# elasticdeeplearning/trainingjob-operator

Hardware: AMD Instinct MI355X
Metric: tokens_per_sec_llama3_8b (higher is better)
Workload: dtype bf16; 1 GPU; model=llama3-8b, global_batch=4, seq_len=4096, parallelism=dp1, micro_batch=2, grad_accum=2, checkpoint_activations=False

## Files before the change

### trainingjob_operator_amd/models/llama.py

```python
from __future__ import annotations

import math
import os
from typing import Optional

import torch
import torch.nn as nn
import torch.nn.functional as F


def _sdpa(q, k, v, enable_gqa=False, is_causal=True):
    backend = os.environ.get("AITJ_SDPA_BACKEND", "auto")
    if q.is_cuda and backend in ("auto", "native") and is_causal:
        from ..ops.attention import _supported, flash_attention
        qc = q.contiguous() if q.stride(-1) != 1 else q
        if _supported(qc, k):
            return flash_attention(qc, k, v)
        if backend == "native":
            groups = q.shape[1] // k.shape[1]
            if groups > 1:
                k = k.repeat_interleave(groups, dim=1)
                v = v.repeat_interleave(groups, dim=1)
            return flash_attention(qc, k, v)
    if backend in ("auto", "native") or not q.is_cuda:
        return F.scaled_dot_product_attention(q, k, v, is_causal=is_causal,
                                              enable_gqa=enable_gqa)
    from torch.nn.attention import SDPBackend, sdpa_kernel
    mapping = {"flash": SDPBackend.FLASH_ATTENTION,
               "efficient": SDPBackend.EFFICIENT_ATTENTION,
               "math": SDPBackend.MATH}
    with sdpa_kernel([mapping[backend]]):
        return F.scaled_dot_product_attention(q, k, v, is_causal=is_causal,
                                              enable_gqa=enable_gqa)

from ..ops import (apply_rope, fused_cross_entropy, fused_rmsnorm,
                   make_inv_freq, swiglu_packed)
from ..ops.fp8 import fp8_enabled, fp8_linear


def _proj(x, linear):
    if fp8_enabled() and x.is_cuda:
        return fp8_linear(x, linear)
    return linear(x)
from .config import LlamaConfig


class Attention(nn.Module):
    def __init__(self, cfg: LlamaConfig):
        super().__init__()
        self.cfg = cfg
        H = cfg.hidden_size
        self.q_size = cfg.num_heads * cfg.head_dim
        self.kv_size = cfg.num_kv_heads * cfg.head_dim
        self.qkv_proj = nn.Linear(H, self.q_size + 2 * self.kv_size,
                                  bias=False)
        self.o_proj = nn.Linear(self.q_size, H, bias=False)

    def forward(self, x: torch.Tensor, inv_freq: torch.Tensor) -> torch.Tensor:
        B, S, H = x.shape
        cfg = self.cfg
        qkv = _proj(x, self.qkv_proj)
        q, k, v = qkv.split([self.q_size, self.kv_size, self.kv_size],
                            dim=-1)
        q = q.reshape(B, S, cfg.num_heads, cfg.head_dim).contiguous()
        k = k.reshape(B, S, cfg.num_kv_heads, cfg.head_dim).contiguous()
        v = v.reshape(B, S, cfg.num_kv_heads, cfg.head_dim)
        q = apply_rope(q, inv_freq, S)
        k = apply_rope(k, inv_freq, S)
        q = q.transpose(1, 2)
        k = k.transpose(1, 2)
        v = v.transpose(1, 2)
        if cfg.num_heads != cfg.num_kv_heads and \
                os.environ.get("AITJ_DISABLE_GQA"):
            groups = cfg.num_heads // cfg.num_kv_heads
            k = k.repeat_interleave(groups, dim=1)
            v = v.repeat_interleave(groups, dim=1)
            o = _sdpa(q, k, v)
        else:
            o = _sdpa(q, k, v,
                      enable_gqa=cfg.num_heads != cfg.num_kv_heads)
        o = o.transpose(1, 2).reshape(B, S, cfg.num_heads * cfg.head_dim)
        return _proj(o, self.o_proj)


class MLP(nn.Module):
    def __init__(self, cfg: LlamaConfig):
        super().__init__()
        H, FF = cfg.hidden_size, cfg.intermediate_size
        self.ff = FF
        self.gate_up_proj = nn.Linear(H, 2 * FF, bias=False)
        self.down_proj = nn.Linear(FF, H, bias=False)

    def forward(self, x: torch.Tensor) -> torch.Tensor:
        return _proj(swiglu_packed(_proj(x, self.gate_up_proj)),
                     self.down_proj)


class Block(nn.Module):
    def __init__(self, cfg: LlamaConfig):
        super().__init__()
        self.cfg = cfg
        self.attn = Attention(cfg)
        self.mlp = MLP(cfg)
        self.input_norm_weight = nn.Parameter(torch.ones(cfg.hidden_size))
        self.post_attn_norm_weight = nn.Parameter(torch.ones(cfg.hidden_size))

    def forward(self, x: torch.Tensor, residual: Optional[torch.Tensor],
                inv_freq: torch.Tensor):
        normed, residual = fused_rmsnorm(x, self.input_norm_weight, residual,
                                         self.cfg.norm_eps)
        attn_out = self.attn(normed, inv_freq)
        normed, residual = fused_rmsnorm(attn_out, self.post_attn_norm_weight,
                                         residual, self.cfg.norm_eps)
        mlp_out = self.mlp(normed)
        return mlp_out, residual


class LlamaModel(nn.Module):
    def __init__(self, cfg: LlamaConfig, checkpoint_activations: bool = False):
        super().__init__()
        self.cfg = cfg
        self.checkpoint_activations = checkpoint_activations
        self.embed = nn.Embedding(cfg.vocab_size, cfg.hidden_size)
        self.blocks = nn.ModuleList(Block(cfg) for _ in range(cfg.num_layers))
        self.final_norm_weight = nn.Parameter(torch.ones(cfg.hidden_size))
        self.lm_head = nn.Linear(cfg.hidden_size, cfg.vocab_size, bias=False)
        if cfg.tie_embeddings:
            self.lm_head.weight = self.embed.weight
        self.register_buffer(
            "inv_freq", make_inv_freq(cfg.head_dim, cfg.rope_theta),
            persistent=False)
        self.reset_parameters()

    def reset_parameters(self):
        std = self.cfg.init_std
        for mod in self.modules():
            if isinstance(mod, (nn.Linear, nn.Embedding)):
                nn.init.normal_(mod.weight, mean=0.0, std=std)
        for name, p in self.named_parameters():
            if name.endswith("norm_weight"):
                nn.init.ones_(p)
        scale = 1.0 / math.sqrt(2 * self.cfg.num_layers)
        for blk in self.blocks:
            nn.init.normal_(blk.attn.o_proj.weight, std=std * scale)
            nn.init.normal_(blk.mlp.down_proj.weight, std=std * scale)

    def forward_hidden(self, tokens: torch.Tensor) -> torch.Tensor:
        x = self.embed(tokens)
        residual = None
        for blk in self.blocks:
            if self.checkpoint_activations and self.training:
                if residual is None:
                    residual = torch.zeros_like(x)
                x, residual = torch.utils.checkpoint.checkpoint(
                    blk, x, residual, self.inv_freq, use_reentrant=False)
            else:
                x, residual = blk(x, residual, self.inv_freq)
        normed, _ = fused_rmsnorm(x, self.final_norm_weight, residual,
                                  self.cfg.norm_eps)
        return normed

    def forward(self, tokens: torch.Tensor,
                targets: Optional[torch.Tensor] = None):
        hidden = self.forward_hidden(tokens)
        logits = self.lm_head(hidden)
        if targets is None:
            return logits
        T = logits.shape[0] * logits.shape[1]
        per_tok = fused_cross_entropy(
            logits.reshape(T, -1).contiguous(), targets.reshape(T))
        n_valid = (targets.reshape(T) != -100).sum().clamp(min=1)
        return per_tok.sum() / n_valid
```

### trainingjob_operator_amd/ops/attention.py

```python
from __future__ import annotations

import math
import os
from typing import Optional

import torch

from . import native


def _supported(q: torch.Tensor, k: torch.Tensor) -> bool:
    B, H, S, D = q.shape
    HKV = k.shape[1]
    return (q.dtype == torch.bfloat16 and D == 128
            and (S % 256 == 0 or (S % 64 == 0 and HKV == H))
            and q.stride(-1) == 1 and k.stride(-1) == 1
            and H % HKV == 0)


def _run_fwd(q, k, v, scale):
    B, H, S, D = q.shape
    HKV = k.shape[1]
    lib = native.load(require=True)
    out = torch.empty(B, H, S, D, dtype=torch.bfloat16, device=q.device)
    lse = torch.empty(B, H, S, dtype=torch.float32, device=q.device)
    rc = lib.attn_fwd(
        native.stream_ptr(), q.data_ptr(), k.data_ptr(), v.data_ptr(),
        out.data_ptr(), lse.data_ptr(),
        q.stride(0), q.stride(1), q.stride(2),
        k.stride(0), k.stride(1), k.stride(2),
        v.stride(0), v.stride(1), v.stride(2),
        B, H, HKV, S, scale)
    native.check_rc(rc, "attn_fwd", f"B={B} H={H} HKV={HKV} S={S}")
    return out, lse


class _NativeFlashAttention(torch.autograd.Function):
    @staticmethod
    def forward(ctx, q, k, v, scale):
        out, lse = _run_fwd(q, k, v, scale)
        ctx.save_for_backward(q, k, v, out, lse)
        ctx.scale = scale
        return out

    @staticmethod
    def backward(ctx, gout):
        q, k, v, out, lse = ctx.saved_tensors
        B, H, S, D = q.shape
        if S % 256 == 0 and os.environ.get("AITJ_ATTN_BWD") != "aten":
            return (*_native_backward(q, k, v, out, lse, gout, ctx.scale),
                    None)
        philox = torch.empty(0, dtype=torch.int64, device=q.device)
        dq, dk, dv = torch.ops.aten._scaled_dot_product_flash_attention_backward(
            gout.contiguous(), q, k, v, out, lse,
            None, None, S, S, 0.0, True,
            philox, philox, scale=ctx.scale)
        return dq, dk, dv, None


def _native_backward(q, k, v, out, lse, gout, scale):
    B, H, S, D = q.shape
    HKV = k.shape[1]
    lib = native.load(require=True)
    dout = gout.contiguous()
    delta = torch.empty(B, H, S, dtype=torch.float32, device=q.device)
    dq = torch.empty(B, H, S, D, dtype=torch.bfloat16, device=q.device)
    dk = torch.empty(B, HKV, S, D, dtype=torch.bfloat16, device=q.device)
    dv = torch.empty(B, HKV, S, D, dtype=torch.bfloat16, device=q.device)
    rc = lib.attn_bwd(
        native.stream_ptr(), q.data_ptr(), k.data_ptr(), v.data_ptr(),
        out.data_ptr(), dout.data_ptr(), lse.data_ptr(), delta.data_ptr(),
        dq.data_ptr(), dk.data_ptr(), dv.data_ptr(),
        q.stride(0), q.stride(1), q.stride(2),
        k.stride(0), k.stride(1), k.stride(2),
        v.stride(0), v.stride(1), v.stride(2),
        B, H, HKV, S, scale)
    native.check_rc(rc, "attn_bwd", f"B={B} H={H} HKV={HKV} S={S}")
    return dq, dk, dv


def flash_attention(q: torch.Tensor, k: torch.Tensor, v: torch.Tensor,
                    scale: Optional[float] = None) -> torch.Tensor:
    if scale is None:
        scale = 1.0 / math.sqrt(q.shape[-1])
    assert _supported(q, k), (
        f"native flash attention needs bf16, D=128, S%256==0 (or S%64==0 "
        f"with equal head counts), d-contiguous strides; got {q.shape} "
        f"{q.dtype} kv={k.shape}")
    return _NativeFlashAttention.apply(q, k, v, scale)


def flash_attention_fwd_only(q, k, v, scale=None):
    if scale is None:
        scale = 1.0 / math.sqrt(q.shape[-1])
    return _run_fwd(q, k, v, scale)


def flash_attention_fwd_nw8(q, k, v, scale=None):
    if scale is None:
        scale = 1.0 / math.sqrt(q.shape[-1])
    B, H, S, D = q.shape
    HKV = k.shape[1]
    lib = native.load(require=True)
    out = torch.empty(B, H, S, D, dtype=torch.bfloat16, device=q.device)
    lse = torch.empty(B, H, S, dtype=torch.float32, device=q.device)
    rc = lib.attn_fwd_nw8(
        native.stream_ptr(), q.data_ptr(), k.data_ptr(), v.data_ptr(),
        out.data_ptr(), lse.data_ptr(),
        q.stride(0), q.stride(1), q.stride(2),
        k.stride(0), k.stride(1), k.stride(2),
        v.stride(0), v.stride(1), v.stride(2),
        B, H, HKV, S, scale)
    native.check_rc(rc, "attn_fwd_nw8", f"B={B} H={H} S={S}")
    return out, lse


def flash_attention_fwd_v7(q, k, v, scale=None):
    if scale is None:
        scale = 1.0 / math.sqrt(q.shape[-1])
    B, H, S, D = q.shape
    HKV = k.shape[1]
    lib = native.load(require=True)
    out = torch.empty(B, H, S, D, dtype=torch.bfloat16, device=q.device)
    lse = torch.empty(B, H, S, dtype=torch.float32, device=q.device)
    rc = lib.attn_fwd_v7(
        native.stream_ptr(), q.data_ptr(), k.data_ptr(), v.data_ptr(),
        out.data_ptr(), lse.data_ptr(),
        q.stride(0), q.stride(1), q.stride(2),
        k.stride(0), k.stride(1), k.stride(2),
        v.stride(0), v.stride(1), v.stride(2),
        B, H, HKV, S, scale)
    native.check_rc(rc, "attn_fwd_v7", f"B={B} H={H} S={S}")
    return out, lse


def flash_attention_fwd_v5(q, k, v, scale=None):
    if scale is None:
        scale = 1.0 / math.sqrt(q.shape[-1])
    B, H, S, D = q.shape
    lib = native.load(require=True)
    out = torch.empty(B, H, S, D, dtype=torch.bfloat16, device=q.device)
    lse = torch.empty(B, H, S, dtype=torch.float32, device=q.device)
    rc = lib.attn_fwd_v5(
        native.stream_ptr(), q.data_ptr(), k.data_ptr(), v.data_ptr(),
        out.data_ptr(), lse.data_ptr(),
        q.stride(0), q.stride(1), q.stride(2),
        k.stride(0), k.stride(1), k.stride(2),
        v.stride(0), v.stride(1), v.stride(2),
        B, H, S, scale)
    native.check_rc(rc, "attn_fwd_v5", f"B={B} H={H} S={S}")
    return out, lse
```

### trainingjob_operator_amd/ops/hip/attention.hip

```cpp

#include <hip/hip_runtime.h>
#include <hip/hip_bf16.h>
#include <cstdint>

typedef unsigned short u16;
typedef unsigned int u32;
typedef __attribute__((ext_vector_type(8))) __bf16 bf16x8;
typedef __attribute__((ext_vector_type(4))) float f32x4;

#define ATTN_BM 64
#define ATTN_BN 64
#define ATTN_D 128
#define ATTN_WAVES 4
__device__ __forceinline__ u16 attn_f2bf(float f) {
  __hip_bfloat16_raw r = __float2bfloat16(f);
  return r.x;
}

__device__ __forceinline__ float bf2f_(u16 b) {
  union { u32 u; float f; } c;
  c.u = ((u32)b) << 16;
  return c.f;
}

__device__ __forceinline__ int k_byte(int row, int col_elem) {
  return (row * ATTN_D * 2 + col_elem * 2) ^ ((row & 15) << 4);
}

#define VT_PITCH_B 144
__device__ __forceinline__ int vt_byte(int d, int kv) {
  const int m = d >> 3;
  return (d * VT_PITCH_B + kv * 2) ^
         ((((m & 7) | (((m >> 1) & 1) << 3))) << 4);
}

__device__ __forceinline__ int p_byte(int row, int col_elem) {
  return (row * ATTN_BN * 2 + col_elem * 2) ^ ((row & 7) << 4);
}

__global__ __launch_bounds__(256) void attn_fwd_kernel(
    const u16* __restrict__ q, const u16* __restrict__ k,
    const u16* __restrict__ v, u16* __restrict__ out,
    float* __restrict__ lse,
    long q_sb, long q_sh, long q_ss,
    long k_sb, long k_sh, long k_ss,
    long v_sb, long v_sh, long v_ss,
    int n_heads, int S, float scale) {
  const int qb = blockIdx.x;
  const int h = blockIdx.y;
  const int b = blockIdx.z;
  const int wid = threadIdx.x >> 6;
  const int lane = threadIdx.x & 63;
  const int low = lane & 15;
  const int kg = lane >> 4;

  __shared__ u16 ldsK[ATTN_BN * ATTN_D];
  __shared__ u16 ldsV[ATTN_D * (VT_PITCH_B / 2) + 128];
  __shared__ u16 ldsP[ATTN_WAVES][16 * ATTN_BN];

  const u16* qbase = q + (long)b * q_sb + (long)h * q_sh
                     + (long)(qb * ATTN_BM) * q_ss;
  union { bf16x8 v; uint4 u; } qfrag[4];
#pragma unroll
  for (int ks = 0; ks < 4; ++ks) {
    qfrag[ks].u = *reinterpret_cast<const uint4*>(
        qbase + (long)(wid * 16 + low) * q_ss + ks * 32 + kg * 8);
  }

  float m_run[4], l_run[4];
  float oacc[8][4];
#pragma unroll
  for (int r = 0; r < 4; ++r) { m_run[r] = -INFINITY; l_run[r] = 0.f; }
#pragma unroll
  for (int ct = 0; ct < 8; ++ct)
#pragma unroll
    for (int r = 0; r < 4; ++r) oacc[ct][r] = 0.f;

  const u16* kbase = k + (long)b * k_sb + (long)h * k_sh;
  const u16* vbase = v + (long)b * v_sb + (long)h * v_sh;
  const int kv_end = (qb + 1) * ATTN_BM;
  char* ldsKb = reinterpret_cast<char*>(ldsK);
  char* ldsVb = reinterpret_cast<char*>(ldsV);
  char* ldsPb = reinterpret_cast<char*>(ldsP[wid]);

  for (int kv0 = 0; kv0 < kv_end; kv0 += ATTN_BN) {
#pragma unroll
    for (int t = 0; t < 4; ++t) {
      const int idx = t * 256 + threadIdx.x;
      const int r = idx >> 4;
      const int c8 = (idx & 15) * 8;
      *reinterpret_cast<uint4*>(&ldsKb[k_byte(r, c8)]) =
          *reinterpret_cast<const uint4*>(
              kbase + (long)(kv0 + r) * k_ss + c8);
      union { uint4 u; u16 h[8]; } vv;
      vv.u = *reinterpret_cast<const uint4*>(
          vbase + (long)(kv0 + r) * v_ss + c8);
#pragma unroll
      for (int j = 0; j < 8; ++j)
        *reinterpret_cast<u16*>(&ldsVb[vt_byte(c8 + j, r)]) = vv.h[j];
    }
    __syncthreads();

    f32x4 sacc[4];
#pragma unroll
    for (int ct = 0; ct < 4; ++ct) {
      f32x4 acc = {0.f, 0.f, 0.f, 0.f};
#pragma unroll
      for (int ks = 0; ks < 4; ++ks) {
        bf16x8 bfrag = *reinterpret_cast<const bf16x8*>(
            &ldsKb[k_byte(ct * 16 + low, ks * 32 + kg * 8)]);
        acc = __builtin_amdgcn_mfma_f32_16x16x32_bf16(qfrag[ks].v, bfrag,
                                                      acc, 0, 0, 0);
      }
      sacc[ct] = acc;
    }

    const int qrow0 = qb * ATTN_BM + wid * 16 + kg * 4;
    float mx[4], alpha[4], psum[4];
#pragma unroll
    for (int r = 0; r < 4; ++r) {
      mx[r] = -INFINITY;
#pragma unroll
      for (int ct = 0; ct < 4; ++ct) {
        const int col = kv0 + ct * 16 + low;
        float s = sacc[ct][r] * scale;
        if (col > qrow0 + r) s = -INFINITY;
        sacc[ct][r] = s;
        mx[r] = fmaxf(mx[r], s);
      }
#pragma unroll
      for (int off = 1; off < 16; off <<= 1)
        mx[r] = fmaxf(mx[r], __shfl_xor(mx[r], off, 64));
      const float mnew = fmaxf(m_run[r], mx[r]);
      alpha[r] = (m_run[r] == -INFINITY) ? 0.f : __expf(m_run[r] - mnew);
      m_run[r] = mnew;
      psum[r] = 0.f;
#pragma unroll
      for (int ct = 0; ct < 4; ++ct) {
        const float p = (sacc[ct][r] == -INFINITY)
                            ? 0.f : __expf(sacc[ct][r] - mnew);
        sacc[ct][r] = p;
        psum[r] += p;
        *reinterpret_cast<u16*>(
            &ldsPb[p_byte(kg * 4 + r, ct * 16 + low)]) = attn_f2bf(p);
      }
#pragma unroll
      for (int off = 1; off < 16; off <<= 1)
        psum[r] += __shfl_xor(psum[r], off, 64);
      l_run[r] = l_run[r] * alpha[r] + psum[r];
#pragma unroll
      for (int ct2 = 0; ct2 < 8; ++ct2) oacc[ct2][r] *= alpha[r];
    }
    __syncthreads();

#pragma unroll
    for (int ct2 = 0; ct2 < 8; ++ct2) {
      f32x4 acc = {oacc[ct2][0], oacc[ct2][1], oacc[ct2][2], oacc[ct2][3]};
#pragma unroll
      for (int ks2 = 0; ks2 < 2; ++ks2) {
        bf16x8 afrag = *reinterpret_cast<const bf16x8*>(
            &ldsPb[p_byte(low, ks2 * 32 + kg * 8)]);
        bf16x8 bfrag = *reinterpret_cast<const bf16x8*>(
            &ldsVb[vt_byte(ct2 * 16 + low, ks2 * 32 + kg * 8)]);
        acc = __builtin_amdgcn_mfma_f32_16x16x32_bf16(afrag, bfrag, acc,
                                                      0, 0, 0);
      }
#pragma unroll
      for (int r = 0; r < 4; ++r) oacc[ct2][r] = acc[r];
    }
    __syncthreads();
  }

  u16* obase = out + (((long)b * n_heads + h) * S + qb * ATTN_BM
                      + wid * 16) * ATTN_D;
#pragma unroll
  for (int r = 0; r < 4; ++r) {
    const float inv_l = 1.0f / l_run[r];
#pragma unroll
    for (int ct2 = 0; ct2 < 8; ++ct2) {
      obase[(long)(kg * 4 + r) * ATTN_D + ct2 * 16 + low] =
          attn_f2bf(oacc[ct2][r] * inv_l);
    }
  }
  if (low == 0) {
    float* lbase = lse + ((long)b * n_heads + h) * S + qb * ATTN_BM
                   + wid * 16 + kg * 4;
#pragma unroll
    for (int r = 0; r < 4; ++r) lbase[r] = m_run[r] + __logf(l_run[r]);
  }
}


typedef __attribute__((ext_vector_type(16))) float f32x16;

#define V6_BM 256
#define V6_QBLK 32
#define V6_BN 64
#define V6_K_U16 (V6_BN * ATTN_D)
#define V6_V_U16 (ATTN_D * (VT_PITCH_B / 2) + 128)
#define V6_BUF_U16 (V6_K_U16 + V6_V_U16)

__device__ __forceinline__ unsigned cvt_pk_bf16(float lo, float hi) {
  unsigned r;
  asm("v_cvt_pk_bf16_f32 %0, %1, %2" : "=v"(r) : "v"(lo), "v"(hi));
  return r;
}

__device__ __forceinline__ float exp2_raw(float x) {
  float r;
  asm("v_exp_f32 %0, %1" : "=v"(r) : "v"(x));
  return r;
}

__device__ __forceinline__ void v7_wait_vmcnt4() {
  asm volatile("s_waitcnt vmcnt(4)" ::: "memory");
}
__device__ __forceinline__ void v7_wait_vmcnt0() {
  asm volatile("s_waitcnt vmcnt(0)" ::: "memory");
}
__device__ __forceinline__ void v7_barrier() {
  asm volatile("s_waitcnt lgkmcnt(0)" ::: "memory");
  __builtin_amdgcn_s_barrier();
}

#define V7_RING 3


template <int NW>
__global__ __launch_bounds__(NW * 64) void attn_fwd_v6_kernel(
    const u16* __restrict__ q, const u16* __restrict__ k,
    const u16* __restrict__ v, u16* __restrict__ out,
    float* __restrict__ lse,
    long q_sb, long q_sh, long q_ss,
    long k_sb, long k_sh, long k_ss,
    long v_sb, long v_sh, long v_ss,
    int n_heads, int gqa_group, int S, float scale2) {
  constexpr int NT = NW * 64;
  constexpr int BM = NW * 32;
  constexpr int KP = 1024 / NT;
  constexpr int VU = 512 / NT;
  const int qb = gridDim.x - 1 - blockIdx.x;
  const int h = blockIdx.y;
  const int b = blockIdx.z;
  const int hkv = h / gqa_group;
  const int tid = threadIdx.x;
  const int wid = tid >> 6;
  const int lane = tid & 63;
  const int low = lane & 31;
  const int hi = lane >> 5;

  __shared__ __attribute__((aligned(16))) u16 lds[2][V6_BUF_U16];

  const int q0w = qb * BM + wid * V6_QBLK;
  const int qrow = q0w + low;

  union F8 { bf16x8 v; uint4 u; u16 h[8]; };
  const u16* qptr = q + (long)b * q_sb + (long)h * q_sh + (long)qrow * q_ss;
  F8 qf[8];
#pragma unroll
  for (int kc = 0; kc < 8; ++kc)
    qf[kc].u = *reinterpret_cast<const uint4*>(qptr + kc * 16 + hi * 8);

  f32x16 oacc[4];
#pragma unroll
  for (int ds = 0; ds < 4; ++ds)
#pragma unroll
    for (int r = 0; r < 16; ++r) oacc[ds][r] = 0.f;
  float m_run = -INFINITY, l_run = 0.f;

  const u16* kbase = k + (long)b * k_sb + (long)hkv * k_sh;
  const u16* vbase = v + (long)b * v_sb + (long)hkv * v_sh;
  const int n_tiles = (qb * BM + BM) / V6_BN;

  char* lds0 = reinterpret_cast<char*>(&lds[0][0]);
  char* lds1 = reinterpret_cast<char*>(&lds[1][0]);
  const int VOFF = V6_K_U16 * 2;

  const u16* kgp[KP];
  const u16* vgp[2 * VU];
#pragma unroll
  for (int i = 0; i < KP; ++i) {
    const int idx = i * NT + tid;
    const int L = idx * 16;
    const int kr = L >> 8;
    const int kin = (((L & 255) ^ ((kr & 15) << 4)) >> 1);
    kgp[i] = kbase + (long)kr * k_ss + kin;
  }
#pragma unroll
  for (int u = 0; u < VU; ++u) {
    const int unit = u * NT + tid;
    const int rp2 = (unit >> 4) * 2;
    const int c8 = (unit & 15) * 8;
#pragma unroll
    for (int i = 0; i < 2; ++i)
      vgp[u * 2 + i] = vbase + (long)(rp2 + i) * v_ss + c8;
  }
  const long kstep = (long)V6_BN * k_ss;
  const long vstep = (long)V6_BN * v_ss;
  const int wu64 = __builtin_amdgcn_readfirstlane(tid >> 6);

  uint4 vst[2 * VU];
#define V6_GLDS_K(BUFI)                                                     \
  _Pragma("unroll")                                                         \
  for (int i = 0; i < KP; ++i) {                                            \
    __builtin_amdgcn_global_load_lds(                                       \
        (const u32*)kgp[i], (u32*)&lds[BUFI][(i * NT + wu64 * 64) * 8],     \
        16, 0, 0);                                                          \
    kgp[i] += kstep;                                                        \
  }
#define V6_LOAD_V()                                                         \
  _Pragma("unroll")                                                         \
  for (int i = 0; i < 2 * VU; ++i) {                                        \
    vst[i] = *reinterpret_cast<const uint4*>(vgp[i]);                       \
    vgp[i] += vstep;                                                        \
  }
#define V6_WRITE_V(BUF)                                                     \
  _Pragma("unroll")                                                         \
  for (int u = 0; u < VU; ++u) {                                            \
    const int unit_ = u * NT + tid;                                         \
    const int rp2_ = (unit_ >> 4) * 2;                                      \
    const int c8_ = (unit_ & 15) * 8;                                       \
    union { uint4 u4; u16 h[8]; } va_, vb_;                                 \
    va_.u4 = vst[u * 2];                                                    \
    vb_.u4 = vst[u * 2 + 1];                                                \
    _Pragma("unroll")                                                       \
    for (int j = 0; j < 8; ++j) {                                           \
      const u32 pair_ = (u32)va_.h[j] | ((u32)vb_.h[j] << 16);              \
      *reinterpret_cast<u32*>(&(BUF)[VOFF + vt_byte(c8_ + j, rp2_)]) = pair_; \
    }                                                                       \
  }

  V6_GLDS_K(0)
  V6_LOAD_V()
  V6_WRITE_V(lds0)
  __syncthreads();

  if (NW == 8 && __builtin_amdgcn_readfirstlane(threadIdx.x) >= NT / 2)
    __builtin_amdgcn_s_setprio(1);

  int cur = 0;
  for (int t = 0; t < n_tiles; ++t) {
    const int kv0 = t * V6_BN;
    const bool have_next = (t + 1) < n_tiles;
    if (have_next) { V6_GLDS_K(cur ^ 1) V6_LOAD_V() }

    char* kb = cur ? lds1 : lds0;
    char* vbuf = kb + VOFF;
    const bool active = kv0 <= q0w + V6_QBLK - 1;
    const bool need_mask = kv0 + V6_BN > q0w;

    f32x16 s0, s1;
    union PF { bf16x8 v; unsigned u[4]; } pa[4];
    float pm = -INFINITY;
    if (active) {
#pragma unroll
      for (int r = 0; r < 16; ++r) { s0[r] = 0.f; s1[r] = 0.f; }
#pragma unroll
      for (int kc = 0; kc < 8; ++kc) {
        bf16x8 a0 = *reinterpret_cast<const bf16x8*>(
            &kb[k_byte(low, kc * 16 + hi * 8)]);
        s0 = __builtin_amdgcn_mfma_f32_32x32x16_bf16(a0, qf[kc].v, s0, 0, 0, 0);
        bf16x8 a1 = *reinterpret_cast<const bf16x8*>(
            &kb[k_byte(32 + low, kc * 16 + hi * 8)]);
        s1 = __builtin_amdgcn_mfma_f32_32x32x16_bf16(a1, qf[kc].v, s1, 0, 0, 0);
      }
      if (need_mask) {
#pragma unroll
        for (int r = 0; r < 16; ++r) {
          const int kvr = kv0 + (r & 3) + 8 * (r >> 2) + 4 * hi;
          float x0 = s0[r] * scale2;
          if (kvr > qrow) x0 = -1e30f;
          s0[r] = x0;
          float x1 = s1[r] * scale2;
          if (kvr + 32 > qrow) x1 = -1e30f;
          s1[r] = x1;
          pm = fmaxf(pm, fmaxf(x0, x1));
        }
      } else {
#pragma unroll
        for (int r = 0; r < 16; ++r) {
          s0[r] *= scale2;
          s1[r] *= scale2;
          pm = fmaxf(pm, fmaxf(s0[r], s1[r]));
        }
      }
      pm = fmaxf(pm, __shfl_xor(pm, 32, 64));
    }
    if (have_next) {
      char* nb = cur ? lds0 : lds1;
      V6_WRITE_V(nb)
    }
    if (active) {
      if (!__all(pm - m_run <= 8.0f)) {
        const float mn = fmaxf(m_run, pm);
        const float alpha = (m_run == -INFINITY) ? 0.f : exp2_raw(m_run - mn);
        m_run = mn;
        l_run *= alpha;
#pragma unroll
        for (int ds = 0; ds < 4; ++ds)
#pragma unroll
          for (int r = 0; r < 16; ++r) oacc[ds][r] *= alpha;
      }
      float psum = 0.f;
#pragma unroll
      for (int r = 0; r < 16; ++r) {
        const float p0 = exp2_raw(s0[r] - m_run);
        const float p1 = exp2_raw(s1[r] - m_run);
        s0[r] = p0;
        s1[r] = p1;
        psum += p0 + p1;
      }
      psum += __shfl_xor(psum, 32, 64);
      l_run += psum;

#pragma unroll
      for (int sub = 0; sub < 2; ++sub) {
#pragma unroll
        for (int cc = 0; cc < 2; ++cc) {
          const int pb = cc * 8;
          unsigned a0, b0, a1, b1;
          if (sub == 0) {
            a0 = cvt_pk_bf16(s0[pb + 0], s0[pb + 1]);
            b0 = cvt_pk_bf16(s0[pb + 4], s0[pb + 5]);
            a1 = cvt_pk_bf16(s0[pb + 2], s0[pb + 3]);
            b1 = cvt_pk_bf16(s0[pb + 6], s0[pb + 7]);
          } else {
            a0 = cvt_pk_bf16(s1[pb + 0], s1[pb + 1]);
            b0 = cvt_pk_bf16(s1[pb + 4], s1[pb + 5]);
            a1 = cvt_pk_bf16(s1[pb + 2], s1[pb + 3]);
            b1 = cvt_pk_bf16(s1[pb + 6], s1[pb + 7]);
          }
          auto r02 = __builtin_amdgcn_permlane32_swap(a0, b0, false, false);
          auto r13 = __builtin_amdgcn_permlane32_swap(a1, b1, false, false);
          PF f;
          f.u[0] = r02[0];
          f.u[1] = r13[0];
          f.u[2] = r02[1];
          f.u[3] = r13[1];
          pa[sub * 2 + cc] = f;
        }
      }

#pragma unroll
      for (int c = 0; c < 4; ++c) {
#pragma unroll
        for (int ds = 0; ds < 4; ++ds) {
          bf16x8 vf = *reinterpret_cast<const bf16x8*>(
              &vbuf[vt_byte(ds * 32 + low, c * 16 + hi * 8)]);
          oacc[ds] = __builtin_amdgcn_mfma_f32_32x32x16_bf16(
              vf, pa[c].v, oacc[ds], 0, 0, 0);
        }
      }
    }
    __syncthreads();
    cur ^= 1;
  }

  const float inv_l = 1.0f / l_run;
  u16* orow = out + (((long)b * n_heads + h) * S + qrow) * ATTN_D;
#pragma unroll
  for (int ds = 0; ds < 4; ++ds) {
#pragma unroll
    for (int g = 0; g < 4; ++g) {
      const int d0 = 8 * g + 4 * hi + 32 * ds;
      const unsigned w0 = cvt_pk_bf16(oacc[ds][4 * g + 0] * inv_l,
                                      oacc[ds][4 * g + 1] * inv_l);
      const unsigned w1 = cvt_pk_bf16(oacc[ds][4 * g + 2] * inv_l,
                                      oacc[ds][4 * g + 3] * inv_l);
      uint2 wv;
      wv.x = w0;
      wv.y = w1;
      *reinterpret_cast<uint2*>(orow + d0) = wv;
    }
  }
  if (hi == 0)
    lse[((long)b * n_heads + h) * S + qrow] =
        m_run * 0.6931471805599453f + __logf(l_run);
}

__global__ __launch_bounds__(512) void attn_fwd_v7_kernel(
    const u16* __restrict__ q, const u16* __restrict__ k,
    const u16* __restrict__ v, u16* __restrict__ out,
    float* __restrict__ lse,
    long q_sb, long q_sh, long q_ss,
    long k_sb, long k_sh, long k_ss,
    long v_sb, long v_sh, long v_ss,
    int n_heads, int gqa_group, int S, float scale2);

extern "C" int attn_fwd(void* stream, const void* q, const void* k,
                        const void* v, void* out, void* lse,
                        long q_sb, long q_sh, long q_ss,
                        long k_sb, long k_sh, long k_ss,
                        long v_sb, long v_sh, long v_ss,
                        int batch, int n_heads, int n_kv_heads, int S,
                        float scale) {
  if (S <= 0 || n_heads <= 0 || batch <= 0 || n_kv_heads <= 0 ||
      n_heads % n_kv_heads != 0)
    return -1;
  if (S % 128 == 0) {
    const float scale2 = scale * 1.4426950408889634f;
    if (S % 256 == 0) {
      dim3 grid(S / 256, n_heads, batch), block(512);
      hipLaunchKernelGGL(attn_fwd_v7_kernel, grid, block, 0,
                         reinterpret_cast<hipStream_t>(stream),
                         (const u16*)q, (const u16*)k, (const u16*)v,
                         (u16*)out, (float*)lse, q_sb, q_sh, q_ss,
                         k_sb, k_sh, k_ss, v_sb, v_sh, v_ss, n_heads,
                         n_heads / n_kv_heads, S, scale2);
      return 0;
    }
    dim3 grid(S / 128, n_heads, batch), block(256);
    hipLaunchKernelGGL((attn_fwd_v6_kernel<4>), grid, block, 0,
                       reinterpret_cast<hipStream_t>(stream),
                       (const u16*)q, (const u16*)k, (const u16*)v, (u16*)out,
                       (float*)lse, q_sb, q_sh, q_ss, k_sb, k_sh, k_ss,
                       v_sb, v_sh, v_ss, n_heads, n_heads / n_kv_heads, S,
                       scale2);
    return 0;
  }
  if (S % ATTN_BM != 0 || n_kv_heads != n_heads) return -1;
  dim3 grid(S / ATTN_BM, n_heads, batch), block(256);
  hipLaunchKernelGGL(attn_fwd_kernel, grid, block, 0,
                     reinterpret_cast<hipStream_t>(stream),
                     (const u16*)q, (const u16*)k, (const u16*)v, (u16*)out,
                     (float*)lse, q_sb, q_sh, q_ss, k_sb, k_sh, k_ss,
                     v_sb, v_sh, v_ss, n_heads, S, scale);
  return 0;
}

extern "C" int attn_fwd_nw8(void* stream, const void* q, const void* k,
                            const void* v, void* out, void* lse,
                            long q_sb, long q_sh, long q_ss,
                            long k_sb, long k_sh, long k_ss,
                            long v_sb, long v_sh, long v_ss,
                            int batch, int n_heads, int n_kv_heads, int S,
                            float scale) {
  if (S <= 0 || S % 256 != 0 || n_heads % n_kv_heads != 0) return -1;
  dim3 grid(S / 256, n_heads, batch), block(512);
  const float scale2 = scale * 1.4426950408889634f;
  hipLaunchKernelGGL((attn_fwd_v6_kernel<8>), grid, block, 0,
                     reinterpret_cast<hipStream_t>(stream),
                     (const u16*)q, (const u16*)k, (const u16*)v, (u16*)out,
                     (float*)lse, q_sb, q_sh, q_ss, k_sb, k_sh, k_ss,
                     v_sb, v_sh, v_ss, n_heads, n_heads / n_kv_heads, S,
                     scale2);
  return 0;
}

extern "C" int attn_fwd_v5(void* stream, const void* q, const void* k,
                           const void* v, void* out, void* lse,
                           long q_sb, long q_sh, long q_ss,
                           long k_sb, long k_sh, long k_ss,
                           long v_sb, long v_sh, long v_ss,
                           int batch, int n_heads, int S, float scale) {
  if (S <= 0 || S % ATTN_BM != 0 || n_heads <= 0 || batch <= 0) return -1;
  dim3 grid(S / ATTN_BM, n_heads, batch), block(256);
  hipLaunchKernelGGL(attn_fwd_kernel, grid, block, 0,
                     reinterpret_cast<hipStream_t>(stream),
                     (const u16*)q, (const u16*)k, (const u16*)v, (u16*)out,
                     (float*)lse, q_sb, q_sh, q_ss, k_sb, k_sh, k_ss,
                     v_sb, v_sh, v_ss, n_heads, S, scale);
  return 0;
}


__global__ __launch_bounds__(256) void attn_delta_kernel(
    const u16* __restrict__ dout, const u16* __restrict__ o,
    float* __restrict__ delta, long n_rows) {
  const long row = (long)blockIdx.x * 16 + (threadIdx.x >> 4);
  if (row >= n_rows) return;
  const int e8 = (threadIdx.x & 15) * 8;
  union { uint4 u; u16 h[8]; } a, b;
  a.u = *reinterpret_cast<const uint4*>(dout + row * ATTN_D + e8);
  b.u = *reinterpret_cast<const uint4*>(o + row * ATTN_D + e8);
  float acc = 0.f;
#pragma unroll
  for (int j = 0; j < 8; ++j)
    acc += bf2f_(a.h[j]) * bf2f_(b.h[j]);
#pragma unroll
  for (int off = 1; off < 16; off <<= 1) acc += __shfl_xor(acc, off, 64);
  if ((threadIdx.x & 15) == 0) delta[row] = acc;
}


#define BQ_K_U16 (V6_BN * ATTN_D)
#define BQ_KT_U16 (ATTN_D * (VT_PITCH_B / 2) + 128)
#define BQ_V_U16 (V6_BN * ATTN_D)
#define BQ_BUF_U16 (BQ_K_U16 + BQ_KT_U16 + BQ_V_U16)

__global__ __launch_bounds__(512) void attn_bwd_dq_kernel(
    const u16* __restrict__ q, const u16* __restrict__ k,
    const u16* __restrict__ v, const u16* __restrict__ dout,
    const float* __restrict__ lse, const float* __restrict__ delta,
    u16* __restrict__ dq,
    long q_sb, long q_sh, long q_ss,
    long k_sb, long k_sh, long k_ss,
    long v_sb, long v_sh, long v_ss,
    int n_heads, int gqa_group, int S, float scale) {
  constexpr int NT = 512;
  const int qb = gridDim.x - 1 - blockIdx.x;
  const int h = blockIdx.y;
  const int b = blockIdx.z;
  const int hkv = h / gqa_group;
  const int tid = threadIdx.x;
  const int wid = tid >> 6;
  const int lane = tid & 63;
  const int low = lane & 31;
  const int hi = lane >> 5;
  const float scale2 = scale * 1.4426950408889634f;

  __shared__ __attribute__((aligned(16))) u16
      lds[V7_RING * 2 * V6_K_U16 + 2 * V6_V_U16];
#define DQ_K(SLOT) (&lds[(SLOT) * V6_K_U16])
#define DQ_VR(SLOT) (&lds[(V7_RING + (SLOT)) * V6_K_U16])
#define DQ_KT(P) (reinterpret_cast<char*>(&lds[2 * V7_RING * V6_K_U16]) \
                  + (P) * (V6_V_U16 * 2))

  const int q0w = qb * 256 + wid * 32;
  const int qrow = q0w + low;

  union F8 { bf16x8 v; uint4 u; u16 h[8]; };
  const u16* qptr = q + (long)b * q_sb + (long)h * q_sh + (long)qrow * q_ss;
  const u16* doptr = dout + (((long)b * n_heads + h) * S + qrow) * ATTN_D;
  F8 qf[8], dof[8];
#pragma unroll
  for (int kc = 0; kc < 8; ++kc) {
    qf[kc].u = *reinterpret_cast<const uint4*>(qptr + kc * 16 + hi * 8);
    dof[kc].u = *reinterpret_cast<const uint4*>(doptr + kc * 16 + hi * 8);
  }
  const long lrow = ((long)b * n_heads + h) * S + qrow;
  const float lse2 = lse[lrow] * 1.4426950408889634f;
  const float dlt = delta[lrow];

  f32x16 dqacc[4];
#pragma unroll
  for (int ds = 0; ds < 4; ++ds)
#pragma unroll
    for (int r = 0; r < 16; ++r) dqacc[ds][r] = 0.f;

  const u16* kbase = k + (long)b * k_sb + (long)hkv * k_sh;
  const u16* vbase = v + (long)b * v_sb + (long)hkv * v_sh;
  const int n_tiles = (qb + 1) * 4;

  const u16* kgp[2];
  const u16* vgp[2];
#pragma unroll
  for (int i = 0; i < 2; ++i) {
    const int L = (tid & ~63) * 32 + i * 1024 + (tid & 63) * 16;
    const int kr = L >> 8;
    const int kin = (((L & 255) ^ ((kr & 15) << 4)) >> 1);
    kgp[i] = kbase + (long)kr * k_ss + kin;
    vgp[i] = vbase + (long)kr * v_ss + kin;
  }
  const long kstep = (long)V6_BN * k_ss;
  const long vstep = (long)V6_BN * v_ss;
  const int lslot = (tid & ~63) * 16;

#define DQ_GLDS(SLOT)                                                       \
  _Pragma("unroll")                                                         \
  for (int i = 0; i < 2; ++i) {                                             \
    __builtin_amdgcn_global_load_lds(                                       \
        (const u32*)kgp[i], (u32*)&DQ_K(SLOT)[i * 512 + lslot],          \
        16, 0, 0);                                                          \
    kgp[i] += kstep;                                                        \
    __builtin_amdgcn_global_load_lds(                                       \
        (const u32*)vgp[i], (u32*)&DQ_VR(SLOT)[i * 512 + lslot],         \
        16, 0, 0);                                                          \
    vgp[i] += vstep;                                                        \
  }

  const int t_rp2 = (tid >> 4) * 2;
  const int t_c8 = (tid & 15) * 8;
#define DQ_TRANSPOSE(SRCSLOT, DST)                                          \
  {                                                                         \
    const char* srcb = reinterpret_cast<const char*>(DQ_K(SRCSLOT));        \
    union { uint4 u4; u16 h[8]; } va_, vb_;                                 \
    va_.u4 = *reinterpret_cast<const uint4*>(&srcb[k_byte(t_rp2, t_c8)]);   \
    vb_.u4 = *reinterpret_cast<const uint4*>(                               \
        &srcb[k_byte(t_rp2 + 1, t_c8)]);                                    \
    _Pragma("unroll")                                                       \
    for (int j = 0; j < 8; ++j) {                                           \
      const u32 pair_ = (u32)va_.h[j] | ((u32)vb_.h[j] << 16);              \
      *reinterpret_cast<u32*>(&(DST)[vt_byte(t_c8 + j, t_rp2)]) = pair_;    \
    }                                                                       \
  }

  DQ_GLDS(0)
  if (n_tiles > 1) DQ_GLDS(1)
  if (n_tiles > 1) v7_wait_vmcnt4(); else v7_wait_vmcnt0();
  v7_barrier();
  DQ_TRANSPOSE(0, DQ_KT(0))
  v7_barrier();

  for (int t = 0; t < n_tiles; ++t) {
    const int kv0 = t * V6_BN;
    const bool have2 = (t + 2) < n_tiles;
    if (have2) DQ_GLDS((t + 2) % V7_RING)

    char* kb = reinterpret_cast<char*>(DQ_K(t % V7_RING));
    char* vb = reinterpret_cast<char*>(DQ_VR(t % V7_RING));
    char* ktb = DQ_KT(t & 1);
    const bool active = kv0 <= q0w + 31;
    const bool need_mask = kv0 + V6_BN > q0w;

    union PF { bf16x8 v; unsigned u[4]; } pds[4];
    if (active) {
#pragma unroll
      for (int sub = 0; sub < 2; ++sub) {
        f32x16 sx, dp;
#pragma unroll
        for (int r = 0; r < 16; ++r) { sx[r] = 0.f; dp[r] = 0.f; }
#pragma unroll
        for (int kc = 0; kc < 8; ++kc) {
          bf16x8 a = *reinterpret_cast<const bf16x8*>(
              &kb[k_byte(sub * 32 + low, kc * 16 + hi * 8)]);
          sx = __builtin_amdgcn_mfma_f32_32x32x16_bf16(a, qf[kc].v, sx,
                                                       0, 0, 0);
          bf16x8 a2 = *reinterpret_cast<const bf16x8*>(
              &vb[k_byte(sub * 32 + low, kc * 16 + hi * 8)]);
          dp = __builtin_amdgcn_mfma_f32_32x32x16_bf16(a2, dof[kc].v, dp,
                                                       0, 0, 0);
        }
#pragma unroll
        for (int r = 0; r < 16; ++r) {
          float x = sx[r] * scale2 - lse2;
          if (need_mask) {
            const int kvr = kv0 + sub * 32 + (r & 3) + 8 * (r >> 2) + 4 * hi;
            if (kvr > qrow) x = -1e30f;
          }
          const float p = exp2_raw(x);
          sx[r] = p * (dp[r] - dlt) * scale;
        }
#pragma unroll
        for (int cc = 0; cc < 2; ++cc) {
          const int pb = cc * 8;
          unsigned a0 = cvt_pk_bf16(sx[pb + 0], sx[pb + 1]);
          unsigned b0 = cvt_pk_bf16(sx[pb + 4], sx[pb + 5]);
          unsigned a1 = cvt_pk_bf16(sx[pb + 2], sx[pb + 3]);
          unsigned b1 = cvt_pk_bf16(sx[pb + 6], sx[pb + 7]);
          auto r02 = __builtin_amdgcn_permlane32_swap(a0, b0, false, false);
          auto r13 = __builtin_amdgcn_permlane32_swap(a1, b1, false, false);
          PF f;
          f.u[0] = r02[0];
          f.u[1] = r13[0];
          f.u[2] = r02[1];
          f.u[3] = r13[1];
          pds[sub * 2 + cc] = f;
        }
      }
#pragma unroll
      for (int c = 0; c < 4; ++c) {
#pragma unroll
        for (int ds = 0; ds < 4; ++ds) {
          bf16x8 kf = *reinterpret_cast<const bf16x8*>(
              &ktb[vt_byte(ds * 32 + low, c * 16 + hi * 8)]);
          dqacc[ds] = __builtin_amdgcn_mfma_f32_32x32x16_bf16(
              kf, pds[c].v, dqacc[ds], 0, 0, 0);
        }
      }
    }
    if (t + 1 < n_tiles) {
      if (have2) v7_wait_vmcnt4(); else v7_wait_vmcnt0();
      DQ_TRANSPOSE((t + 1) % V7_RING, DQ_KT((t + 1) & 1))
    }
    v7_barrier();
  }

  u16* dqrow = dq + (((long)b * n_heads + h) * S + qrow) * ATTN_D;
#pragma unroll
  for (int ds = 0; ds < 4; ++ds) {
#pragma unroll
    for (int g = 0; g < 4; ++g) {
      const int d0 = 8 * g + 4 * hi + 32 * ds;
      const unsigned w0 = cvt_pk_bf16(dqacc[ds][4 * g + 0],
                                      dqacc[ds][4 * g + 1]);
      const unsigned w1 = cvt_pk_bf16(dqacc[ds][4 * g + 2],
                                      dqacc[ds][4 * g + 3]);
      uint2 wv;
      wv.x = w0;
      wv.y = w1;
      *reinterpret_cast<uint2*>(dqrow + d0) = wv;
    }
  }
}


#define BV_Q_U16 (V6_BN * ATTN_D)
#define BV_DOT_U16 (ATTN_D * (VT_PITCH_B / 2) + 128)
#define BV_LSE_U16 128
#define BV_BUF_U16 (BV_Q_U16 + BV_DOT_U16 + BV_LSE_U16)

__global__ __launch_bounds__(512) void attn_bwd_dv_kernel(
    const u16* __restrict__ q, const u16* __restrict__ k,
    const u16* __restrict__ dout, const float* __restrict__ lse,
    u16* __restrict__ dv,
    long q_sb, long q_sh, long q_ss,
    long k_sb, long k_sh, long k_ss,
    int n_heads, int n_kv_heads, int S, float scale) {
  const int kvb = blockIdx.x;
  const int hkv = blockIdx.y;
  const int b = blockIdx.z;
  const int gqa_group = n_heads / n_kv_heads;
  const int tid = threadIdx.x;
  const int wid = tid >> 6;
  const int lane = tid & 63;
  const int low = lane & 31;
  const int hi = lane >> 5;
  const float scale2 = scale * 1.4426950408889634f;

  __shared__ __attribute__((aligned(16))) u16 lds[2][BV_BUF_U16];
  char* lds0 = reinterpret_cast<char*>(&lds[0][0]);
  char* lds1 = reinterpret_cast<char*>(&lds[1][0]);
  const int DOTOFF = BV_Q_U16 * 2;
  const int LSEOFF = (BV_Q_U16 + BV_DOT_U16) * 2;

  const int kv0w = kvb * 256 + wid * 32;
  const int kvrow = kv0w + low;

  union F8 { bf16x8 v; uint4 u; u16 h[8]; };
  const u16* kptr = k + (long)b * k_sb + (long)hkv * k_sh + (long)kvrow * k_ss;
  F8 kf[8];
#pragma unroll
  for (int kc = 0; kc < 8; ++kc)
    kf[kc].u = *reinterpret_cast<const uint4*>(kptr + kc * 16 + hi * 8);

  f32x16 dvacc[4];
#pragma unroll
  for (int ds = 0; ds < 4; ++ds)
#pragma unroll
    for (int r = 0; r < 16; ++r) dvacc[ds][r] = 0.f;

  const int qt0 = kvb * 4;
  const int qtn = S / 64;
  const int wu64 = __builtin_amdgcn_readfirstlane(tid >> 6);
  uint4 dtst[2];

  for (int g = 0; g < gqa_group; ++g) {
    const int h = hkv * gqa_group + g;
    const u16* qbase = q + (long)b * q_sb + (long)h * q_sh;
    const u16* dobase = dout + (((long)b * n_heads + h) * S) * ATTN_D;
    const float* lbase = lse + ((long)b * n_heads + h) * S;

    const u16* qgp[2];
    const u16* dtp[2];
    {
      const int idx0 = tid, idx1 = 512 + tid;
      const int L0 = idx0 * 16, L1 = idx1 * 16;
      const int r0 = L0 >> 8, r1 = L1 >> 8;
      const int in0 = (((L0 & 255) ^ ((r0 & 15) << 4)) >> 1);
      const int in1 = (((L1 & 255) ^ ((r1 & 15) << 4)) >> 1);
      qgp[0] = qbase + (long)(qt0 * 64 + r0) * q_ss + in0;
      qgp[1] = qbase + (long)(qt0 * 64 + r1) * q_ss + in1;
      const int rp2 = (tid >> 4) * 2;
      const int c8 = (tid & 15) * 8;
      dtp[0] = dobase + (long)(qt0 * 64 + rp2) * ATTN_D + c8;
      dtp[1] = dobase + (long)(qt0 * 64 + rp2 + 1) * ATTN_D + c8;
    }
    const long qstep = (long)64 * q_ss;
    const long dostep = (long)64 * ATTN_D;

#define BV_STAGE_IN(BUFI, QT)                                               \
    {                                                                       \
      _Pragma("unroll")                                                     \
      for (int i = 0; i < 2; ++i) {                                         \
        __builtin_amdgcn_global_load_lds(                                   \
            (const u32*)qgp[i], (u32*)&lds[BUFI][(i * 512 + wu64 * 64) * 8],\
            16, 0, 0);                                                      \
        qgp[i] += qstep;                                                    \
      }                                                                     \
      dtst[0] = *reinterpret_cast<const uint4*>(dtp[0]);                    \
      dtst[1] = *reinterpret_cast<const uint4*>(dtp[1]);                    \
      dtp[0] += dostep;                                                     \
      dtp[1] += dostep;                                                     \
      if (tid < 64)                                                         \
        *reinterpret_cast<float*>(                                          \
            &lds[BUFI][LSEOFF / 2 + tid * 2]) =                             \
            lbase[(QT) * 64 + tid] * 1.4426950408889634f;                   \
    }
#define BV_WRITE_DOT(BUF)                                                   \
    {                                                                       \
      const int rp2_ = (tid >> 4) * 2;                                      \
      const int c8_ = (tid & 15) * 8;                                       \
      union { uint4 u4; u16 h[8]; } va_, vb_;                               \
      va_.u4 = dtst[0];                                                     \
      vb_.u4 = dtst[1];                                                     \
      _Pragma("unroll")                                                     \
      for (int j = 0; j < 8; ++j) {                                         \
        const u32 pair_ = (u32)va_.h[j] | ((u32)vb_.h[j] << 16);            \
        *reinterpret_cast<u32*>(&(BUF)[DOTOFF + vt_byte(c8_ + j, rp2_)]) =  \
            pair_;                                                          \
      }                                                                     \
    }

    BV_STAGE_IN(0, qt0)
    BV_WRITE_DOT(lds0)
    __syncthreads();

    int cur = 0;
    for (int qt = qt0; qt < qtn; ++qt) {
      const bool have_next = (qt + 1) < qtn;
      if (have_next) BV_STAGE_IN(cur ^ 1, qt + 1)

      char* qb_ = cur ? lds1 : lds0;
      char* dob = qb_ + DOTOFF;
      const float* lse2t = reinterpret_cast<const float*>(qb_ + LSEOFF);
      const bool active = qt * 64 + 63 >= kv0w;
      const bool need_mask = qt * 64 < kv0w + 32;

      union PF { bf16x8 v; unsigned u[4]; } pf[4];
      if (active) {
#pragma unroll
        for (int sub = 0; sub < 2; ++sub) {
          f32x16 s;
#pragma unroll
          for (int r = 0; r < 16; ++r) s[r] = 0.f;
#pragma unroll
          for (int kc = 0; kc < 8; ++kc) {
            bf16x8 a = *reinterpret_cast<const bf16x8*>(
                &qb_[k_byte(sub * 32 + low, kc * 16 + hi * 8)]);
            s = __builtin_amdgcn_mfma_f32_32x32x16_bf16(a, kf[kc].v, s,
                                                        0, 0, 0);
          }
#pragma unroll
          for (int r = 0; r < 16; ++r) {
            const int qr = (r & 3) + 8 * (r >> 2) + 4 * hi;
            float x = s[r] * scale2 - lse2t[sub * 32 + qr];
            if (need_mask && qt * 64 + sub * 32 + qr < kvrow) x = -1e30f;
            s[r] = exp2_raw(x);
          }
#pragma unroll
          for (int cc = 0; cc < 2; ++cc) {
            const int pb = cc * 8;
            unsigned a0 = cvt_pk_bf16(s[pb + 0], s[pb + 1]);
            unsigned b0 = cvt_pk_bf16(s[pb + 4], s[pb + 5]);
            unsigned a1 = cvt_pk_bf16(s[pb + 2], s[pb + 3]);
            unsigned b1 = cvt_pk_bf16(s[pb + 6], s[pb + 7]);
            auto r02 = __builtin_amdgcn_permlane32_swap(a0, b0, false, false);
            auto r13 = __builtin_amdgcn_permlane32_swap(a1, b1, false, false);
            PF f;
            f.u[0] = r02[0];
            f.u[1] = r13[0];
            f.u[2] = r02[1];
            f.u[3] = r13[1];
            pf[sub * 2 + cc] = f;
          }
        }
      }
      if (have_next) {
        char* nb = cur ? lds0 : lds1;
        BV_WRITE_DOT(nb)
      }
      if (active) {
#pragma unroll
        for (int c = 0; c < 4; ++c) {
#pragma unroll
          for (int ds = 0; ds < 4; ++ds) {
            bf16x8 af = *reinterpret_cast<const bf16x8*>(
                &dob[vt_byte(ds * 32 + low, c * 16 + hi * 8)]);
            dvacc[ds] = __builtin_amdgcn_mfma_f32_32x32x16_bf16(
                af, pf[c].v, dvacc[ds], 0, 0, 0);
          }
        }
      }
      __syncthreads();
      cur ^= 1;
    }
  }

  u16* dvrow = dv + (((long)b * n_kv_heads + hkv) * S + kvrow) * ATTN_D;
#pragma unroll
  for (int ds = 0; ds < 4; ++ds) {
#pragma unroll
    for (int g = 0; g < 4; ++g) {
      const int d0 = 8 * g + 4 * hi + 32 * ds;
      const unsigned w0 = cvt_pk_bf16(dvacc[ds][4 * g + 0],
                                      dvacc[ds][4 * g + 1]);
      const unsigned w1 = cvt_pk_bf16(dvacc[ds][4 * g + 2],
                                      dvacc[ds][4 * g + 3]);
      uint2 wv;
      wv.x = w0;
      wv.y = w1;
      *reinterpret_cast<uint2*>(dvrow + d0) = wv;
    }
  }
}


#define BK_Q_U16 (V6_BN * ATTN_D)
#define BK_DO_U16 (V6_BN * ATTN_D)
#define BK_QT_U16 (ATTN_D * (VT_PITCH_B / 2) + 128)
#define BK_LSE_U16 128
#define BK_DLT_U16 128
#define BK_BUF_U16 (BK_Q_U16 + BK_DO_U16 + BK_QT_U16 + BK_LSE_U16 + BK_DLT_U16)

__global__ __launch_bounds__(512) void attn_bwd_dk_kernel(
    const u16* __restrict__ q, const u16* __restrict__ k,
    const u16* __restrict__ v, const u16* __restrict__ dout,
    const float* __restrict__ lse, const float* __restrict__ delta,
    u16* __restrict__ dk,
    long q_sb, long q_sh, long q_ss,
    long k_sb, long k_sh, long k_ss,
    long v_sb, long v_sh, long v_ss,
    int n_heads, int n_kv_heads, int S, float scale) {
  const int kvb = blockIdx.x;
  const int hkv = blockIdx.y;
  const int b = blockIdx.z;
  const int gqa_group = n_heads / n_kv_heads;
  const int tid = threadIdx.x;
  const int wid = tid >> 6;
  const int lane = tid & 63;
  const int low = lane & 31;
  const int hi = lane >> 5;
  const float scale2 = scale * 1.4426950408889634f;

  __shared__ __attribute__((aligned(16))) u16 lds[2][BK_BUF_U16];
  char* lds0 = reinterpret_cast<char*>(&lds[0][0]);
  char* lds1 = reinterpret_cast<char*>(&lds[1][0]);
  const int DOOFF = BK_Q_U16 * 2;
  const int QTOFF = (BK_Q_U16 + BK_DO_U16) * 2;
  const int LSEOFF = (BK_Q_U16 + BK_DO_U16 + BK_QT_U16) * 2;
  const int DLTOFF = LSEOFF + BK_LSE_U16 * 2;

  const int kv0w = kvb * 256 + wid * 32;
  const int kvrow = kv0w + low;

  union F8 { bf16x8 v; uint4 u; u16 h[8]; };
  const u16* kptr = k + (long)b * k_sb + (long)hkv * k_sh + (long)kvrow * k_ss;
  const u16* vptr = v + (long)b * v_sb + (long)hkv * v_sh + (long)kvrow * v_ss;
  F8 kf[8], vf[8];
#pragma unroll
  for (int kc = 0; kc < 8; ++kc) {
    kf[kc].u = *reinterpret_cast<const uint4*>(kptr + kc * 16 + hi * 8);
    vf[kc].u = *reinterpret_cast<const uint4*>(vptr + kc * 16 + hi * 8);
  }

  f32x16 dkacc[4];
#pragma unroll
  for (int ds = 0; ds < 4; ++ds)
#pragma unroll
    for (int r = 0; r < 16; ++r) dkacc[ds][r] = 0.f;

  const int qt0 = kvb * 4;
  const int qtn = S / 64;
  const int wu64 = __builtin_amdgcn_readfirstlane(tid >> 6);
  uint4 qtst[2];

  for (int g = 0; g < gqa_group; ++g) {
    const int h = hkv * gqa_group + g;
    const u16* qbase = q + (long)b * q_sb + (long)h * q_sh;
    const u16* dobase = dout + (((long)b * n_heads + h) * S) * ATTN_D;
    const float* lbase = lse + ((long)b * n_heads + h) * S;
    const float* dbase = delta + ((long)b * n_heads + h) * S;

    const u16* qgp[2];
    const u16* dgp[2];
    const u16* qtp[2];
    {
      const int idx0 = tid, idx1 = 512 + tid;
      const int L0 = idx0 * 16, L1 = idx1 * 16;
      const int r0 = L0 >> 8, r1 = L1 >> 8;
      const int in0 = (((L0 & 255) ^ ((r0 & 15) << 4)) >> 1);
      const int in1 = (((L1 & 255) ^ ((r1 & 15) << 4)) >> 1);
      qgp[0] = qbase + (long)(qt0 * 64 + r0) * q_ss + in0;
      qgp[1] = qbase + (long)(qt0 * 64 + r1) * q_ss + in1;
      dgp[0] = dobase + (long)(qt0 * 64 + r0) * ATTN_D + in0;
      dgp[1] = dobase + (long)(qt0 * 64 + r1) * ATTN_D + in1;
      const int rp2 = (tid >> 4) * 2;
      const int c8 = (tid & 15) * 8;
      qtp[0] = qbase + (long)(qt0 * 64 + rp2) * q_ss + c8;
      qtp[1] = qbase + (long)(qt0 * 64 + rp2 + 1) * q_ss + c8;
    }
    const long qstep = (long)64 * q_ss;
    const long dostep = (long)64 * ATTN_D;

#define BK_STAGE_IN(BUFI, QT)                                               \
    {                                                                       \
      _Pragma("unroll")                                                     \
      for (int i = 0; i < 2; ++i) {                                         \
        __builtin_amdgcn_global_load_lds(                                   \
            (const u32*)qgp[i], (u32*)&lds[BUFI][(i * 512 + wu64 * 64) * 8],\
            16, 0, 0);                                                      \
        qgp[i] += qstep;                                                    \
        __builtin_amdgcn_global_load_lds(                                   \
            (const u32*)dgp[i],                                             \
            (u32*)&lds[BUFI][DOOFF / 2 + (i * 512 + wu64 * 64) * 8],        \
            16, 0, 0);                                                      \
        dgp[i] += dostep;                                                   \
      }                                                                     \
      qtst[0] = *reinterpret_cast<const uint4*>(qtp[0]);                    \
      qtst[1] = *reinterpret_cast<const uint4*>(qtp[1]);                    \
      qtp[0] += qstep;                                                      \
      qtp[1] += qstep;                                                      \
      if (tid < 64)                                                         \
        *reinterpret_cast<float*>(&lds[BUFI][LSEOFF / 2 + tid * 2]) =       \
            lbase[(QT) * 64 + tid] * 1.4426950408889634f;                   \
      else if (tid < 128)                                                   \
        *reinterpret_cast<float*>(                                          \
            &lds[BUFI][DLTOFF / 2 + (tid - 64) * 2]) =                      \
            dbase[(QT) * 64 + tid - 64];                                    \
    }
#define BK_WRITE_QT(BUF)                                                    \
    {                                                                       \
      const int rp2_ = (tid >> 4) * 2;                                      \
      const int c8_ = (tid & 15) * 8;                                       \
      union { uint4 u4; u16 h[8]; } va_, vb_;                               \
      va_.u4 = qtst[0];                                                     \
      vb_.u4 = qtst[1];                                                     \
      _Pragma("unroll")                                                     \
      for (int j = 0; j < 8; ++j) {                                         \
        const u32 pair_ = (u32)va_.h[j] | ((u32)vb_.h[j] << 16);            \
        *reinterpret_cast<u32*>(&(BUF)[QTOFF + vt_byte(c8_ + j, rp2_)]) =   \
            pair_;                                                          \
      }                                                                     \
    }

    BK_STAGE_IN(0, qt0)
    BK_WRITE_QT(lds0)
    __syncthreads();

    int cur = 0;
    for (int qt = qt0; qt < qtn; ++qt) {
      const bool have_next = (qt + 1) < qtn;
      if (have_next) BK_STAGE_IN(cur ^ 1, qt + 1)

      char* qb_ = cur ? lds1 : lds0;
      char* dob = qb_ + DOOFF;
      char* qtb = qb_ + QTOFF;
      const float* lse2t = reinterpret_cast<const float*>(qb_ + LSEOFF);
      const float* dltt = reinterpret_cast<const float*>(qb_ + DLTOFF);
      const bool active = qt * 64 + 63 >= kv0w;
      const bool need_mask = qt * 64 < kv0w + 32;

      union PF { bf16x8 v; unsigned u[4]; } pf[4];
      if (active) {
#pragma unroll
        for (int sub = 0; sub < 2; ++sub) {
          f32x16 s, dp;
#pragma unroll
          for (int r = 0; r < 16; ++r) { s[r] = 0.f; dp[r] = 0.f; }
#pragma unroll
          for (int kc = 0; kc < 8; ++kc) {
            bf16x8 a = *reinterpret_cast<const bf16x8*>(
                &qb_[k_byte(sub * 32 + low, kc * 16 + hi * 8)]);
            s = __builtin_amdgcn_mfma_f32_32x32x16_bf16(a, kf[kc].v, s,
                                                        0, 0, 0);
            bf16x8 a2 = *reinterpret_cast<const bf16x8*>(
                &dob[k_byte(sub * 32 + low, kc * 16 + hi * 8)]);
            dp = __builtin_amdgcn_mfma_f32_32x32x16_bf16(a2, vf[kc].v, dp,
                                                         0, 0, 0);
          }
#pragma unroll
          for (int r = 0; r < 16; ++r) {
            const int qr = (r & 3) + 8 * (r >> 2) + 4 * hi;
            float x = s[r] * scale2 - lse2t[sub * 32 + qr];
            if (need_mask && qt * 64 + sub * 32 + qr < kvrow) x = -1e30f;
            const float p = exp2_raw(x);
            s[r] = p * (dp[r] - dltt[sub * 32 + qr]) * scale;
          }
#pragma unroll
          for (int cc = 0; cc < 2; ++cc) {
            const int pb = cc * 8;
            unsigned a0 = cvt_pk_bf16(s[pb + 0], s[pb + 1]);
            unsigned b0 = cvt_pk_bf16(s[pb + 4], s[pb + 5]);
            unsigned a1 = cvt_pk_bf16(s[pb + 2], s[pb + 3]);
            unsigned b1 = cvt_pk_bf16(s[pb + 6], s[pb + 7]);
            auto r02 = __builtin_amdgcn_permlane32_swap(a0, b0, false, false);
            auto r13 = __builtin_amdgcn_permlane32_swap(a1, b1, false, false);
            PF f;
            f.u[0] = r02[0];
            f.u[1] = r13[0];
            f.u[2] = r02[1];
            f.u[3] = r13[1];
            pf[sub * 2 + cc] = f;
          }
        }
      }
      if (have_next) {
        char* nb = cur ? lds0 : lds1;
        BK_WRITE_QT(nb)
      }
      if (active) {
#pragma unroll
        for (int c = 0; c < 4; ++c) {
#pragma unroll
          for (int ds = 0; ds < 4; ++ds) {
            bf16x8 af = *reinterpret_cast<const bf16x8*>(
                &qtb[vt_byte(ds * 32 + low, c * 16 + hi * 8)]);
            dkacc[ds] = __builtin_amdgcn_mfma_f32_32x32x16_bf16(
                af, pf[c].v, dkacc[ds], 0, 0, 0);
          }
        }
      }
      __syncthreads();
      cur ^= 1;
    }
  }

  u16* dkrow = dk + (((long)b * n_kv_heads + hkv) * S + kvrow) * ATTN_D;
#pragma unroll
  for (int ds = 0; ds < 4; ++ds) {
#pragma unroll
    for (int g = 0; g < 4; ++g) {
      const int d0 = 8 * g + 4 * hi + 32 * ds;
      const unsigned w0 = cvt_pk_bf16(dkacc[ds][4 * g + 0],
                                      dkacc[ds][4 * g + 1]);
      const unsigned w1 = cvt_pk_bf16(dkacc[ds][4 * g + 2],
                                      dkacc[ds][4 * g + 3]);
      uint2 wv;
      wv.x = w0;
      wv.y = w1;
      *reinterpret_cast<uint2*>(dkrow + d0) = wv;
    }
  }
}




extern "C" int attn_bwd(void* stream, const void* q, const void* k,
                        const void* v, const void* out, const void* dout,
                        const void* lse, void* delta,
                        void* dq, void* dk, void* dv,
                        long q_sb, long q_sh, long q_ss,
                        long k_sb, long k_sh, long k_ss,
                        long v_sb, long v_sh, long v_ss,
                        int batch, int n_heads, int n_kv_heads, int S,
                        float scale) {
  if (S <= 0 || S % 256 != 0 || n_heads <= 0 || batch <= 0 ||
      n_kv_heads <= 0 || n_heads % n_kv_heads != 0)
    return -1;
  hipStream_t st = reinterpret_cast<hipStream_t>(stream);
  const long n_rows = (long)batch * n_heads * S;
  hipLaunchKernelGGL(attn_delta_kernel,
                     dim3((unsigned)((n_rows + 15) / 16)), dim3(256), 0, st,
                     (const u16*)dout, (const u16*)out, (float*)delta,
                     n_rows);
  {
    dim3 grid(S / 256, n_heads, batch), block(512);
    hipLaunchKernelGGL(attn_bwd_dq_kernel, grid, block, 0, st,
                       (const u16*)q, (const u16*)k, (const u16*)v,
                       (const u16*)dout, (const float*)lse,
                       (const float*)delta, (u16*)dq,
                       q_sb, q_sh, q_ss, k_sb, k_sh, k_ss,
                       v_sb, v_sh, v_ss, n_heads, n_heads / n_kv_heads, S,
                       scale);
  }
  {
    dim3 grid(S / 256, n_kv_heads, batch), block(512);
    hipLaunchKernelGGL(attn_bwd_dv_kernel, grid, block, 0, st,
                       (const u16*)q, (const u16*)k, (const u16*)dout,
                       (const float*)lse, (u16*)dv,
                       q_sb, q_sh, q_ss, k_sb, k_sh, k_ss,
                       n_heads, n_kv_heads, S, scale);
    hipLaunchKernelGGL(attn_bwd_dk_kernel, grid, block, 0, st,
                       (const u16*)q, (const u16*)k, (const u16*)v,
                       (const u16*)dout, (const float*)lse,
                       (const float*)delta, (u16*)dk,
                       q_sb, q_sh, q_ss, k_sb, k_sh, k_ss,
                       v_sb, v_sh, v_ss, n_heads, n_kv_heads, S, scale);
  }
  return 0;
}


__global__ __launch_bounds__(512) void attn_fwd_v7_kernel(
    const u16* __restrict__ q, const u16* __restrict__ k,
    const u16* __restrict__ v, u16* __restrict__ out,
    float* __restrict__ lse,
    long q_sb, long q_sh, long q_ss,
    long k_sb, long k_sh, long k_ss,
    long v_sb, long v_sh, long v_ss,
    int n_heads, int gqa_group, int S, float scale2) {
  constexpr int NT = 512;
  const int qb = gridDim.x - 1 - blockIdx.x;
  const int h = blockIdx.y;
  const int b = blockIdx.z;
  const int hkv = h / gqa_group;
  const int tid = threadIdx.x;
  const int wid = tid >> 6;
  const int lane = tid & 63;
  const int low = lane & 31;
  const int hi = lane >> 5;

  __shared__ __attribute__((aligned(16))) u16
      lds[V7_RING * 2 * V6_K_U16 + 2 * V6_V_U16];
#define LDSK(SLOT) (&lds[(SLOT) * V6_K_U16])
#define LDSVR(SLOT) (&lds[(V7_RING + (SLOT)) * V6_K_U16])
#define LDSVT(P) (reinterpret_cast<char*>(&lds[2 * V7_RING * V6_K_U16]) \
                  + (P) * (V6_V_U16 * 2))

  const int q0w = qb * 256 + wid * 32;
  const int qrow = q0w + low;

  union F8 { bf16x8 v; uint4 u; u16 h[8]; };
  const u16* qptr = q + (long)b * q_sb + (long)h * q_sh + (long)qrow * q_ss;
  F8 qf[8];
#pragma unroll
  for (int kc = 0; kc < 8; ++kc)
    qf[kc].u = *reinterpret_cast<const uint4*>(qptr + kc * 16 + hi * 8);

  f32x16 oacc[4];
#pragma unroll
  for (int ds = 0; ds < 4; ++ds)
#pragma unroll
    for (int r = 0; r < 16; ++r) oacc[ds][r] = 0.f;
  float m_run = -INFINITY, l_run = 0.f;

  const u16* kbase = k + (long)b * k_sb + (long)hkv * k_sh;
  const u16* vbase = v + (long)b * v_sb + (long)hkv * v_sh;
  const int n_tiles = (qb + 1) * 4;

  const u16* kgp[2];
  const u16* vgp[2];
#pragma unroll
  for (int i = 0; i < 2; ++i) {
    const int L = (tid & ~63) * 32 + i * 1024 + (tid & 63) * 16;
    const int kr = L >> 8;
    const int kin = (((L & 255) ^ ((kr & 15) << 4)) >> 1);
    kgp[i] = kbase + (long)kr * k_ss + kin;
    vgp[i] = vbase + (long)kr * v_ss + kin;
  }
  const long kstep = (long)V6_BN * k_ss;
  const long vstep = (long)V6_BN * v_ss;
  const int lslot = (tid & ~63) * 16;

#define V7_GLDS(SLOT)                                                       \
  _Pragma("unroll")                                                         \
  for (int i = 0; i < 2; ++i) {                                             \
    __builtin_amdgcn_global_load_lds(                                       \
        (const u32*)kgp[i], (u32*)&LDSK(SLOT)[i * 512 + lslot],          \
        16, 0, 0);                                                          \
    kgp[i] += kstep;                                                        \
    __builtin_amdgcn_global_load_lds(                                       \
        (const u32*)vgp[i], (u32*)&LDSVR(SLOT)[i * 512 + lslot],         \
        16, 0, 0);                                                          \
    vgp[i] += vstep;                                                        \
  }

  const int t_rp2 = (tid >> 4) * 2;
  const int t_c8 = (tid & 15) * 8;
#define V7_TRANSPOSE(SRCSLOT, DST)                                          \
  {                                                                         \
    const char* srcb = reinterpret_cast<const char*>(LDSVR(SRCSLOT));       \
    union { uint4 u4; u16 h[8]; } va_, vb_;                                 \
    va_.u4 = *reinterpret_cast<const uint4*>(&srcb[k_byte(t_rp2, t_c8)]);   \
    vb_.u4 = *reinterpret_cast<const uint4*>(                               \
        &srcb[k_byte(t_rp2 + 1, t_c8)]);                                    \
    _Pragma("unroll")                                                       \
    for (int j = 0; j < 8; ++j) {                                           \
      const u32 pair_ = (u32)va_.h[j] | ((u32)vb_.h[j] << 16);              \
      *reinterpret_cast<u32*>(&(DST)[vt_byte(t_c8 + j, t_rp2)]) = pair_;    \
    }                                                                       \
  }

  V7_GLDS(0)
  if (n_tiles > 1) V7_GLDS(1)
  if (n_tiles > 1) v7_wait_vmcnt4(); else v7_wait_vmcnt0();
  v7_barrier();
  V7_TRANSPOSE(0, LDSVT(0))
  v7_barrier();

  for (int t = 0; t < n_tiles; ++t) {
    const int kv0 = t * V6_BN;
    const bool have2 = (t + 2) < n_tiles;
    if (have2) V7_GLDS((t + 2) % V7_RING)

    char* kb = reinterpret_cast<char*>(LDSK(t % V7_RING));
    char* vtb = LDSVT(t & 1);
    const bool active = kv0 <= q0w + 31;
    const bool need_mask = kv0 + V6_BN > q0w;

    f32x16 s0, s1;
    union PF { bf16x8 v; unsigned u[4]; } pa[4];
    float pm = -INFINITY;
    if (active) {
#pragma unroll
      for (int r = 0; r < 16; ++r) { s0[r] = 0.f; s1[r] = 0.f; }
#pragma unroll
      for (int kc = 0; kc < 8; ++kc) {
        bf16x8 a0 = *reinterpret_cast<const bf16x8*>(
            &kb[k_byte(low, kc * 16 + hi * 8)]);
        s0 = __builtin_amdgcn_mfma_f32_32x32x16_bf16(a0, qf[kc].v, s0, 0, 0, 0);
        bf16x8 a1 = *reinterpret_cast<const bf16x8*>(
            &kb[k_byte(32 + low, kc * 16 + hi * 8)]);
        s1 = __builtin_amdgcn_mfma_f32_32x32x16_bf16(a1, qf[kc].v, s1, 0, 0, 0);
      }
      if (need_mask) {
#pragma unroll
        for (int r = 0; r < 16; ++r) {
          const int kvr = kv0 + (r & 3) + 8 * (r >> 2) + 4 * hi;
          float x0 = s0[r] * scale2;
          if (kvr > qrow) x0 = -1e30f;
          s0[r] = x0;
          float x1 = s1[r] * scale2;
          if (kvr + 32 > qrow) x1 = -1e30f;
          s1[r] = x1;
          pm = fmaxf(pm, fmaxf(x0, x1));
        }
      } else {
#pragma unroll
        for (int r = 0; r < 16; ++r) {
          s0[r] *= scale2;
          s1[r] *= scale2;
          pm = fmaxf(pm, fmaxf(s0[r], s1[r]));
        }
      }
      pm = fmaxf(pm, __shfl_xor(pm, 32, 64));

      if (!__all(pm - m_run <= 8.0f)) {
        const float mn = fmaxf(m_run, pm);
        const float alpha = (m_run == -INFINITY) ? 0.f : exp2_raw(m_run - mn);
        m_run = mn;
        l_run *= alpha;
#pragma unroll
        for (int ds = 0; ds < 4; ++ds)
#pragma unroll
          for (int r = 0; r < 16; ++r) oacc[ds][r] *= alpha;
      }
      float psum = 0.f;
#pragma unroll
      for (int r = 0; r < 16; ++r) {
        const float p0 = exp2_raw(s0[r] - m_run);
        const float p1 = exp2_raw(s1[r] - m_run);
        s0[r] = p0;
        s1[r] = p1;
        psum += p0 + p1;
      }
      psum += __shfl_xor(psum, 32, 64);
      l_run += psum;

#pragma unroll
      for (int sub = 0; sub < 2; ++sub) {
#pragma unroll
        for (int cc = 0; cc < 2; ++cc) {
          const int pb = cc * 8;
          unsigned a0, b0, a1, b1;
          if (sub == 0) {
            a0 = cvt_pk_bf16(s0[pb + 0], s0[pb + 1]);
            b0 = cvt_pk_bf16(s0[pb + 4], s0[pb + 5]);
            a1 = cvt_pk_bf16(s0[pb + 2], s0[pb + 3]);
            b1 = cvt_pk_bf16(s0[pb + 6], s0[pb + 7]);
          } else {
            a0 = cvt_pk_bf16(s1[pb + 0], s1[pb + 1]);
            b0 = cvt_pk_bf16(s1[pb + 4], s1[pb + 5]);
            a1 = cvt_pk_bf16(s1[pb + 2], s1[pb + 3]);
            b1 = cvt_pk_bf16(s1[pb + 6], s1[pb + 7]);
          }
          auto r02 = __builtin_amdgcn_permlane32_swap(a0, b0, false, false);
          auto r13 = __builtin_amdgcn_permlane32_swap(a1, b1, false, false);
          PF f;
          f.u[0] = r02[0];
          f.u[1] = r13[0];
          f.u[2] = r02[1];
          f.u[3] = r13[1];
          pa[sub * 2 + cc] = f;
        }
      }

#pragma unroll
      for (int c = 0; c < 4; ++c) {
#pragma unroll
        for (int ds = 0; ds < 4; ++ds) {
          bf16x8 vf = *reinterpret_cast<const bf16x8*>(
              &vtb[vt_byte(ds * 32 + low, c * 16 + hi * 8)]);
          oacc[ds] = __builtin_amdgcn_mfma_f32_32x32x16_bf16(
              vf, pa[c].v, oacc[ds], 0, 0, 0);
        }
      }
    }
    if (t + 1 < n_tiles) {
      if (have2) v7_wait_vmcnt4(); else v7_wait_vmcnt0();
      V7_TRANSPOSE((t + 1) % V7_RING, LDSVT((t + 1) & 1))
    }
    v7_barrier();
  }

  const float inv_l = 1.0f / l_run;
  u16* orow = out + (((long)b * n_heads + h) * S + qrow) * ATTN_D;
#pragma unroll
  for (int ds = 0; ds < 4; ++ds) {
#pragma unroll
    for (int g = 0; g < 4; ++g) {
      const int d0 = 8 * g + 4 * hi + 32 * ds;
      const unsigned w0 = cvt_pk_bf16(oacc[ds][4 * g + 0] * inv_l,
                                      oacc[ds][4 * g + 1] * inv_l);
      const unsigned w1 = cvt_pk_bf16(oacc[ds][4 * g + 2] * inv_l,
                                      oacc[ds][4 * g + 3] * inv_l);
      uint2 wv;
      wv.x = w0;
      wv.y = w1;
      *reinterpret_cast<uint2*>(orow + d0) = wv;
    }
  }
  if (hi == 0)
    lse[((long)b * n_heads + h) * S + qrow] =
        m_run * 0.6931471805599453f + __logf(l_run);
}

extern "C" int attn_fwd_v7(void* stream, const void* q, const void* k,
                           const void* v, void* out, void* lse,
                           long q_sb, long q_sh, long q_ss,
                           long k_sb, long k_sh, long k_ss,
                           long v_sb, long v_sh, long v_ss,
                           int batch, int n_heads, int n_kv_heads, int S,
                           float scale) {
  if (S <= 0 || S % 256 != 0 || n_heads % n_kv_heads != 0) return -1;
  dim3 grid(S / 256, n_heads, batch), block(512);
  const float scale2 = scale * 1.4426950408889634f;
  hipLaunchKernelGGL(attn_fwd_v7_kernel, grid, block, 0,
                     reinterpret_cast<hipStream_t>(stream),
                     (const u16*)q, (const u16*)k, (const u16*)v, (u16*)out,
                     (float*)lse, q_sb, q_sh, q_ss, k_sb, k_sh, k_ss,
                     v_sb, v_sh, v_ss, n_heads, n_heads / n_kv_heads, S,
                     scale2);
  return 0;
}
```

### trainingjob_operator_amd/ops/hip/ops.hip

```cpp

#include <hip/hip_runtime.h>
#include <hip/hip_bf16.h>
#include <cstdint>
#include <cstdio>

#define WAVE 64
#define BLOCK 256
#define WAVES_PER_BLOCK (BLOCK / WAVE)

typedef unsigned short u16;
typedef unsigned int u32;


union BF8 {
  uint4 v;
  u16 h[8];
};

__device__ __forceinline__ float bf2f(u16 b) {
  union { u32 u; float f; } c;
  c.u = ((u32)b) << 16;
  return c.f;
}

__device__ __forceinline__ u16 f2bf(float f) {
  __hip_bfloat16_raw r = __float2bfloat16(f);
  return r.x;
}


__device__ __forceinline__ float wave_reduce_sum(float v) {
#pragma unroll
  for (int off = 32; off > 0; off >>= 1) v += __shfl_xor(v, off, WAVE);
  return v;
}

__device__ __forceinline__ float block_reduce_sum(float v, float* lds) {
  v = wave_reduce_sum(v);
  const int lane = threadIdx.x & (WAVE - 1);
  const int wid = threadIdx.x >> 6;
  if (lane == 0) lds[wid] = v;
  __syncthreads();
  float total = 0.f;
#pragma unroll
  for (int w = 0; w < WAVES_PER_BLOCK; ++w) total += lds[w];
  __syncthreads();
  return total;
}


template <int NITER>
__global__ void rmsnorm_fwd_kernel(
    const uint4* __restrict__ x, const uint4* __restrict__ res_in,
    const uint4* __restrict__ w, uint4* __restrict__ y,
    uint4* __restrict__ res_out, float* __restrict__ rrms_out,
    int H8, float eps) {
  __shared__ float lds[WAVES_PER_BLOCK];
  const long row = blockIdx.x;
  const uint4* xr = x + row * H8;
  const uint4* rr = res_in ? res_in + row * H8 : nullptr;
  uint4* yr = y + row * H8;
  uint4* ror = res_out ? res_out + row * H8 : nullptr;

  float vals[NITER][8];
  float sumsq = 0.f;
#pragma unroll
  for (int it = 0; it < NITER; ++it) {
    const int idx = it * BLOCK + threadIdx.x;
    BF8 a; a.v = xr[idx];
#pragma unroll
    for (int j = 0; j < 8; ++j) vals[it][j] = bf2f(a.h[j]);
    if (rr) {
      BF8 b; b.v = rr[idx];
#pragma unroll
      for (int j = 0; j < 8; ++j) vals[it][j] += bf2f(b.h[j]);
      BF8 o;
#pragma unroll
      for (int j = 0; j < 8; ++j) o.h[j] = f2bf(vals[it][j]);
      ror[idx] = o.v;
#pragma unroll
      for (int j = 0; j < 8; ++j) vals[it][j] = bf2f(o.h[j]);
    }
#pragma unroll
    for (int j = 0; j < 8; ++j) sumsq += vals[it][j] * vals[it][j];
  }
  const int H = H8 * 8;
  const float total = block_reduce_sum(sumsq, lds);
  const float rrms = rsqrtf(total / (float)H + eps);
  if (threadIdx.x == 0 && rrms_out) rrms_out[row] = rrms;

#pragma unroll
  for (int it = 0; it < NITER; ++it) {
    const int idx = it * BLOCK + threadIdx.x;
    BF8 wv; wv.v = w[idx];
    BF8 o;
#pragma unroll
    for (int j = 0; j < 8; ++j) o.h[j] = f2bf(vals[it][j] * rrms * bf2f(wv.h[j]));
    yr[idx] = o.v;
  }
}


#define DW_ROWS 4

template <int NITER>
__global__ void rmsnorm_bwd_kernel(
    const uint4* __restrict__ dy, const uint4* __restrict__ res_out,
    const uint4* __restrict__ w, const float* __restrict__ rrms_in,
    const uint4* __restrict__ dres, uint4* __restrict__ dx,
    float* __restrict__ dw_partial, long n_rows, int H8) {
  __shared__ float lds[WAVES_PER_BLOCK];
  const int H = H8 * 8;
  float wv[NITER][8];
#pragma unroll
  for (int it = 0; it < NITER; ++it) {
    BF8 a; a.v = w[it * BLOCK + threadIdx.x];
#pragma unroll
    for (int j = 0; j < 8; ++j) wv[it][j] = bf2f(a.h[j]);
  }
  float dwacc[NITER][8] = {};

  const long row0 = (long)blockIdx.x * DW_ROWS;
  for (long row = row0; row < row0 + DW_ROWS && row < n_rows; ++row) {
    const uint4* dyr = dy + row * H8;
    const uint4* xr = res_out + row * H8;
    uint4* dxr = dx + row * H8;
    const float rrms = rrms_in[row];

    float xv[NITER][8], dxh[NITER][8], dyv[NITER][8];
    float dot = 0.f;
#pragma unroll
    for (int it = 0; it < NITER; ++it) {
      const int idx = it * BLOCK + threadIdx.x;
      BF8 a; a.v = xr[idx];
      BF8 d; d.v = dyr[idx];
#pragma unroll
      for (int j = 0; j < 8; ++j) {
        xv[it][j] = bf2f(a.h[j]);
        dyv[it][j] = bf2f(d.h[j]);
        dxh[it][j] = dyv[it][j] * wv[it][j];
        dot += dxh[it][j] * xv[it][j];
      }
    }
    const float rr = rrms;
    const float m = block_reduce_sum(dot, lds) * rr * rr / (float)H;
#pragma unroll
    for (int it = 0; it < NITER; ++it) {
      const int idx = it * BLOCK + threadIdx.x;
      BF8 o;
      if (dres) {
        BF8 dr; dr.v = dres[row * H8 + idx];
#pragma unroll
        for (int j = 0; j < 8; ++j)
          o.h[j] = f2bf(rr * (dxh[it][j] - xv[it][j] * m) + bf2f(dr.h[j]));
      } else {
#pragma unroll
        for (int j = 0; j < 8; ++j)
          o.h[j] = f2bf(rr * (dxh[it][j] - xv[it][j] * m));
      }
      dxr[idx] = o.v;
#pragma unroll
      for (int j = 0; j < 8; ++j) dwacc[it][j] += dyv[it][j] * xv[it][j] * rr;
    }
  }
  float* dwp = dw_partial + (long)blockIdx.x * H;
#pragma unroll
  for (int it = 0; it < NITER; ++it) {
    const int idx = it * BLOCK + threadIdx.x;
#pragma unroll
    for (int j = 0; j < 8; ++j) dwp[idx * 8 + j] = dwacc[it][j];
  }
}


__global__ void rmsnorm_fwd_generic_kernel(
    const uint4* __restrict__ x, const uint4* __restrict__ res_in,
    const uint4* __restrict__ w, uint4* __restrict__ y,
    uint4* __restrict__ res_out, float* __restrict__ rrms_out,
    int H8, float eps) {
  __shared__ float lds[WAVES_PER_BLOCK];
  const long row = blockIdx.x;
  const uint4* xr = x + row * H8;
  const uint4* rr = res_in ? res_in + row * H8 : nullptr;
  uint4* yr = y + row * H8;
  uint4* ror = res_out ? res_out + row * H8 : nullptr;

  float sumsq = 0.f;
  for (int idx = threadIdx.x; idx < H8; idx += BLOCK) {
    BF8 a; a.v = xr[idx];
    float vals[8];
#pragma unroll
    for (int j = 0; j < 8; ++j) vals[j] = bf2f(a.h[j]);
    if (rr) {
      BF8 b; b.v = rr[idx];
#pragma unroll
      for (int j = 0; j < 8; ++j) vals[j] += bf2f(b.h[j]);
      BF8 o;
#pragma unroll
      for (int j = 0; j < 8; ++j) o.h[j] = f2bf(vals[j]);
      ror[idx] = o.v;
#pragma unroll
      for (int j = 0; j < 8; ++j) vals[j] = bf2f(o.h[j]);
    }
#pragma unroll
    for (int j = 0; j < 8; ++j) sumsq += vals[j] * vals[j];
  }
  const float total = block_reduce_sum(sumsq, lds);
  const float rrms = rsqrtf(total / (float)(H8 * 8) + eps);
  if (threadIdx.x == 0 && rrms_out) rrms_out[row] = rrms;

  const uint4* src = rr ? (const uint4*)ror : xr;
  for (int idx = threadIdx.x; idx < H8; idx += BLOCK) {
    BF8 a; a.v = src[idx];
    BF8 wv; wv.v = w[idx];
    BF8 o;
#pragma unroll
    for (int j = 0; j < 8; ++j)
      o.h[j] = f2bf(bf2f(a.h[j]) * rrms * bf2f(wv.h[j]));
    yr[idx] = o.v;
  }
}

__global__ void rmsnorm_bwd_generic_kernel(
    const uint4* __restrict__ dy, const uint4* __restrict__ res_out,
    const uint4* __restrict__ w, const float* __restrict__ rrms_in,
    const uint4* __restrict__ dres, uint4* __restrict__ dx,
    float* __restrict__ dw_partial, int H8) {
  __shared__ float lds[WAVES_PER_BLOCK];
  const long row = blockIdx.x;
  const int H = H8 * 8;
  const uint4* dyr = dy + row * H8;
  const uint4* xr = res_out + row * H8;
  uint4* dxr = dx + row * H8;
  const float rr = rrms_in[row];

  float dot = 0.f;
  for (int idx = threadIdx.x; idx < H8; idx += BLOCK) {
    BF8 a; a.v = xr[idx];
    BF8 d; d.v = dyr[idx];
    BF8 wv; wv.v = w[idx];
#pragma unroll
    for (int j = 0; j < 8; ++j)
      dot += bf2f(d.h[j]) * bf2f(wv.h[j]) * bf2f(a.h[j]);
  }
  const float m = block_reduce_sum(dot, lds) * rr * rr / (float)H;
  float* dwp = dw_partial + row * (long)H;
  for (int idx = threadIdx.x; idx < H8; idx += BLOCK) {
    BF8 a; a.v = xr[idx];
    BF8 d; d.v = dyr[idx];
    BF8 wv; wv.v = w[idx];
    BF8 o;
    if (dres) {
      BF8 dr; dr.v = dres[row * H8 + idx];
#pragma unroll
      for (int j = 0; j < 8; ++j)
        o.h[j] = f2bf(rr * (bf2f(d.h[j]) * bf2f(wv.h[j])
                            - bf2f(a.h[j]) * m) + bf2f(dr.h[j]));
    } else {
#pragma unroll
      for (int j = 0; j < 8; ++j)
        o.h[j] = f2bf(rr * (bf2f(d.h[j]) * bf2f(wv.h[j])
                            - bf2f(a.h[j]) * m));
    }
    dxr[idx] = o.v;
#pragma unroll
    for (int j = 0; j < 8; ++j)
      dwp[idx * 8 + j] = bf2f(d.h[j]) * bf2f(a.h[j]) * rr;
  }
}

__global__ void rmsnorm_dw_reduce_kernel(float* __restrict__ dw_partial,
                                         int n_partials,
                                         float* __restrict__ dw_out, int H,
                                         int rows_per_block, int row_step) {
  const int h = blockIdx.x * blockDim.x + threadIdx.x;
  if (h >= H) return;
  const int p0 = blockIdx.y * rows_per_block;
  int p1 = p0 + rows_per_block;
  if (p1 > n_partials) p1 = n_partials;
  float acc = 0.f;
  for (int p = p0; p < p1; p += row_step) acc += dw_partial[(long)p * H + h];
  if (dw_out) dw_out[h] = acc;
  else if (p0 < n_partials) dw_partial[(long)p0 * H + h] = acc;
}


__global__ void rope_kernel(const uint4* __restrict__ x, uint4* __restrict__ out,
                            const float* __restrict__ inv_freq,
                            long total_vec, int vec_per_half, int n_heads,
                            int S, int D, float sign, int pos0,
                            const long* __restrict__ pos_dev) {
  const int HALF = D / 2;
  for (long g = blockIdx.x * (long)blockDim.x + threadIdx.x; g < total_vec;
       g += gridDim.x * (long)blockDim.x) {
    const long per_head = vec_per_half;
    const long head_g = g / per_head;
    const int i0 = (int)(g % per_head) * 8;
    const long t = head_g / n_heads;
    const int h = (int)(head_g % n_heads);
    const int pos = pos0 + (int)(t % S) + (pos_dev ? (int)*pos_dev : 0);
    const long base = (t * n_heads + h) * (D / 8);
    BF8 a; a.v = x[base + i0 / 8];
    BF8 b; b.v = x[base + (HALF + i0) / 8];
    BF8 oa, ob;
#pragma unroll
    for (int j = 0; j < 8; ++j) {
      float c, s;
      __sincosf((float)pos * inv_freq[i0 + j], &s, &c);
      s *= sign;
      const float x1 = bf2f(a.h[j]), x2 = bf2f(b.h[j]);
      oa.h[j] = f2bf(x1 * c - x2 * s);
      ob.h[j] = f2bf(x1 * s + x2 * c);
    }
    out[base + i0 / 8] = oa.v;
    out[base + (HALF + i0) / 8] = ob.v;
  }
}


__device__ __forceinline__ float sigmoidf_fast(float x) {
  return 1.0f / (1.0f + __expf(-x));
}

__global__ void swiglu_fwd_kernel(const uint4* __restrict__ g,
                                  const uint4* __restrict__ u,
                                  uint4* __restrict__ out, long n8) {
  for (long i = blockIdx.x * (long)blockDim.x + threadIdx.x; i < n8;
       i += gridDim.x * (long)blockDim.x) {
    BF8 gv, uv, ov;
    gv.v = g[i]; uv.v = u[i];
#pragma unroll
    for (int j = 0; j < 8; ++j) {
      const float gf = bf2f(gv.h[j]);
      ov.h[j] = f2bf(gf * sigmoidf_fast(gf) * bf2f(uv.h[j]));
    }
    out[i] = ov.v;
  }
}

__global__ void swiglu_packed_fwd_kernel(const uint4* __restrict__ gu,
                                         uint4* __restrict__ out,
                                         long n_rows, int F8) {
  const long total = n_rows * F8;
  for (long i = blockIdx.x * (long)blockDim.x + threadIdx.x; i < total;
       i += gridDim.x * (long)blockDim.x) {
    const long row = i / F8;
    const int col = (int)(i % F8);
    BF8 gv, uv, ov;
    gv.v = gu[row * 2 * F8 + col];
    uv.v = gu[row * 2 * F8 + F8 + col];
#pragma unroll
    for (int j = 0; j < 8; ++j) {
      const float gf = bf2f(gv.h[j]);
      ov.h[j] = f2bf(gf * sigmoidf_fast(gf) * bf2f(uv.h[j]));
    }
    out[i] = ov.v;
  }
}

__global__ void swiglu_packed_bwd_kernel(const uint4* __restrict__ dout,
                                         const uint4* __restrict__ gu,
                                         uint4* __restrict__ dgu,
                                         long n_rows, int F8) {
  const long total = n_rows * F8;
  for (long i = blockIdx.x * (long)blockDim.x + threadIdx.x; i < total;
       i += gridDim.x * (long)blockDim.x) {
    const long row = i / F8;
    const int col = (int)(i % F8);
    BF8 dov, gv, uv, dgv, duv;
    dov.v = dout[i];
    gv.v = gu[row * 2 * F8 + col];
    uv.v = gu[row * 2 * F8 + F8 + col];
#pragma unroll
    for (int j = 0; j < 8; ++j) {
      const float dof = bf2f(dov.h[j]);
      const float gf = bf2f(gv.h[j]);
      const float sg = sigmoidf_fast(gf);
      duv.h[j] = f2bf(dof * gf * sg);
      dgv.h[j] = f2bf(dof * bf2f(uv.h[j]) * sg * (1.f + gf * (1.f - sg)));
    }
    dgu[row * 2 * F8 + col] = dgv.v;
    dgu[row * 2 * F8 + F8 + col] = duv.v;
  }
}

__global__ void swiglu_bwd_kernel(const uint4* __restrict__ dout,
                                  const uint4* __restrict__ g,
                                  const uint4* __restrict__ u,
                                  uint4* __restrict__ dg,
                                  uint4* __restrict__ du, long n8) {
  for (long i = blockIdx.x * (long)blockDim.x + threadIdx.x; i < n8;
       i += gridDim.x * (long)blockDim.x) {
    BF8 dov, gv, uv, dgv, duv;
    dov.v = dout[i]; gv.v = g[i]; uv.v = u[i];
#pragma unroll
    for (int j = 0; j < 8; ++j) {
      const float dof = bf2f(dov.h[j]);
      const float gf = bf2f(gv.h[j]);
      const float sg = sigmoidf_fast(gf);
      const float silu = gf * sg;
      duv.h[j] = f2bf(dof * silu);
      dgv.h[j] = f2bf(dof * bf2f(uv.h[j]) * sg * (1.f + gf * (1.f - sg)));
    }
    dg[i] = dgv.v;
    du[i] = duv.v;
  }
}


__device__ __forceinline__ void online_combine(float& m, float& s, float m2, float s2) {
  const float mm = fmaxf(m, m2);
  if (mm == -INFINITY) { s = 0.f; m = mm; return; }
  s = s * __expf(m - mm) + s2 * __expf(m2 - mm);
  m = mm;
}

__global__ void ce_fwd_kernel(const uint4* __restrict__ logits,
                              const int* __restrict__ targets,
                              float* __restrict__ lse_out,
                              float* __restrict__ loss_out,
                              int V, int ignore_index) {
  __shared__ float lds_m[WAVES_PER_BLOCK];
  __shared__ float lds_s[WAVES_PER_BLOCK];
  const long row = blockIdx.x;
  const int V8 = V / 8;
  const uint4* lr = logits + row * V8;

  float m = -INFINITY, s = 0.f;
  for (int i = threadIdx.x; i < V8; i += BLOCK) {
    BF8 a; a.v = lr[i];
#pragma unroll
    for (int j = 0; j < 8; ++j) {
      const float x = bf2f(a.h[j]);
      if (x > m) { s *= __expf(m - x); m = x; }
      s += __expf(x - m);
    }
  }
#pragma unroll
  for (int off = 32; off > 0; off >>= 1) {
    const float m2 = __shfl_xor(m, off, WAVE);
    const float s2 = __shfl_xor(s, off, WAVE);
    online_combine(m, s, m2, s2);
  }
  const int lane = threadIdx.x & (WAVE - 1);
  const int wid = threadIdx.x >> 6;
  if (lane == 0) { lds_m[wid] = m; lds_s[wid] = s; }
  __syncthreads();
  if (threadIdx.x == 0) {
    float M = lds_m[0], S = lds_s[0];
#pragma unroll
    for (int w = 1; w < WAVES_PER_BLOCK; ++w) online_combine(M, S, lds_m[w], lds_s[w]);
    const float lse = M + __logf(S);
    lse_out[row] = lse;
    const int t = targets[row];
    if (t == ignore_index) {
      loss_out[row] = 0.f;
    } else {
      const u16* lrow = reinterpret_cast<const u16*>(lr);
      loss_out[row] = lse - bf2f(lrow[t]);
    }
  }
}

__global__ void ce_bwd_kernel(const uint4* __restrict__ logits,
                              const int* __restrict__ targets,
                              const float* __restrict__ lse,
                              const float* __restrict__ gscale,
                              uint4* __restrict__ dlogits,
                              int V, int ignore_index) {
  const long row = blockIdx.x;
  const int V8 = V / 8;
  const uint4* lr = logits + row * V8;
  uint4* dr = dlogits + row * V8;
  const int t = targets[row];
  const float l = lse[row];
  const float gs = (t == ignore_index) ? 0.f : gscale[row];
  for (int i = threadIdx.x; i < V8; i += BLOCK) {
    BF8 a; a.v = lr[i];
    BF8 o;
#pragma unroll
    for (int j = 0; j < 8; ++j) {
      const int col = i * 8 + j;
      float p = __expf(bf2f(a.h[j]) - l);
      if (col == t) p -= 1.f;
      o.h[j] = f2bf(p * gs);
    }
    dr[i] = o.v;
  }
}


__global__ void rows_gather_kernel(const uint4* __restrict__ in,
                                   const long* __restrict__ idx,
                                   uint4* __restrict__ out,
                                   long n_out, int H8) {
  const long total = n_out * H8;
  for (long g = blockIdx.x * (long)blockDim.x + threadIdx.x; g < total;
       g += gridDim.x * (long)blockDim.x) {
    const long i = g / H8;
    const int h = (int)(g % H8);
    out[g] = in[idx[i] * H8 + h];
  }
}

__global__ void rows_scatter_kernel(const uint4* __restrict__ in,
                                    const long* __restrict__ idx,
                                    uint4* __restrict__ out,
                                    long n_in, int H8) {
  const long total = n_in * H8;
  for (long g = blockIdx.x * (long)blockDim.x + threadIdx.x; g < total;
       g += gridDim.x * (long)blockDim.x) {
    const long i = g / H8;
    const int h = (int)(g % H8);
    out[idx[i] * H8 + h] = in[g];
  }
}

__global__ void rows_scatter_add_f32_kernel(const uint4* __restrict__ in,
                                            const long* __restrict__ idx,
                                            float* __restrict__ accum,
                                            long n_in, int H8) {
  const long total = n_in * H8;
  for (long g = blockIdx.x * (long)blockDim.x + threadIdx.x; g < total;
       g += gridDim.x * (long)blockDim.x) {
    const long i = g / H8;
    const int h = (int)(g % H8);
    BF8 a; a.v = in[g];
    float* dst = accum + (idx[i] * (long)H8 + h) * 8;
#pragma unroll
    for (int j = 0; j < 8; ++j) atomicAdd(&dst[j], bf2f(a.h[j]));
  }
}

__global__ void moe_combine_kernel(const uint4* __restrict__ src,
                                   const long* __restrict__ inv,
                                   const float* __restrict__ gates,
                                   uint4* __restrict__ y,
                                   long T, int K, int H8) {
  const long total = T * H8;
  for (long g = blockIdx.x * (long)blockDim.x + threadIdx.x; g < total;
       g += gridDim.x * (long)blockDim.x) {
    const long t = g / H8;
    const int h = (int)(g % H8);
    float acc[8] = {};
    for (int j = 0; j < K; ++j) {
      const long row = inv[t * K + j];
      const float gj = gates ? gates[t * K + j] : 1.0f;
      BF8 a; a.v = src[row * H8 + h];
#pragma unroll
      for (int m = 0; m < 8; ++m) acc[m] += gj * bf2f(a.h[m]);
    }
    BF8 o;
#pragma unroll
    for (int m = 0; m < 8; ++m) o.h[m] = f2bf(acc[m]);
    y[g] = o.v;
  }
}

__global__ void moe_combine_bwd_dsrc_kernel(const uint4* __restrict__ dy,
                                            const long* __restrict__ inv,
                                            const float* __restrict__ gates,
                                            uint4* __restrict__ dsrc,
                                            long n_pairs, int K, int H8) {
  const long total = n_pairs * H8;
  for (long g = blockIdx.x * (long)blockDim.x + threadIdx.x; g < total;
       g += gridDim.x * (long)blockDim.x) {
    const long pair = g / H8;
    const int h = (int)(g % H8);
    const long row = inv[pair];
    const float gj = gates[pair];
    BF8 d; d.v = dy[(pair / K) * H8 + h];
    BF8 o;
#pragma unroll
    for (int m = 0; m < 8; ++m) o.h[m] = f2bf(gj * bf2f(d.h[m]));
    dsrc[row * H8 + h] = o.v;
  }
}

__global__ void moe_combine_bwd_dgate_kernel(const uint4* __restrict__ src,
                                             const uint4* __restrict__ dy,
                                             const long* __restrict__ inv,
                                             float* __restrict__ dgate,
                                             long n_pairs, int K, int H8) {
  const long pair = blockIdx.x * (long)(BLOCK / 16) + (threadIdx.x >> 4);
  if (pair >= n_pairs) return;
  const long row = inv[pair];
  const long t = pair / K;
  float acc = 0.f;
  for (int h = threadIdx.x & 15; h < H8; h += 16) {
    BF8 a; a.v = src[row * H8 + h];
    BF8 d; d.v = dy[t * H8 + h];
#pragma unroll
    for (int m = 0; m < 8; ++m) acc += bf2f(a.h[m]) * bf2f(d.h[m]);
  }
#pragma unroll
  for (int off = 1; off < 16; off <<= 1) acc += __shfl_xor(acc, off, 64);
  if ((threadIdx.x & 15) == 0) dgate[pair] = acc;
}


__global__ void l2normsq_partial_kernel(const uint4* __restrict__ grad, long n8,
                                        float* __restrict__ partials) {
  __shared__ float lds[WAVES_PER_BLOCK];
  float acc = 0.f;
  for (long i = blockIdx.x * (long)blockDim.x + threadIdx.x; i < n8;
       i += gridDim.x * (long)blockDim.x) {
    BF8 a; a.v = grad[i];
#pragma unroll
    for (int j = 0; j < 8; ++j) {
      const float x = bf2f(a.h[j]);
      acc += x * x;
    }
  }
  acc = block_reduce_sum(acc, lds);
  if (threadIdx.x == 0) partials[blockIdx.x] = acc;
}

__global__ void reduce_partials_kernel(const float* __restrict__ partials, int n,
                                       float* __restrict__ out) {
  __shared__ float lds[WAVES_PER_BLOCK];
  float acc = 0.f;
  for (int i = threadIdx.x; i < n; i += BLOCK) acc += partials[i];
  acc = block_reduce_sum(acc, lds);
  if (threadIdx.x == 0) out[0] = acc;
}

__global__ void adamw_kernel(float* __restrict__ p32, float* __restrict__ m,
                             float* __restrict__ v, const uint2* __restrict__ grad,
                             uint2* __restrict__ p_bf16,
                             const float* __restrict__ normsq, long n4,
                             float lr, float beta1, float beta2, float eps,
                             float weight_decay, float bc1, float bc2,
                             float clip, float pre_scale,
                             const float* __restrict__ bc_dev) {
  if (bc_dev) { bc1 = bc_dev[0]; bc2 = bc_dev[1]; }
  float gscale = pre_scale;
  if (normsq) {
    const float norm = sqrtf(*normsq) * pre_scale;
    gscale = pre_scale * (clip / fmaxf(clip, norm));
  }
  float4* p4 = reinterpret_cast<float4*>(p32);
  float4* m4 = reinterpret_cast<float4*>(m);
  float4* v4 = reinterpret_cast<float4*>(v);
  for (long i = blockIdx.x * (long)blockDim.x + threadIdx.x; i < n4;
       i += gridDim.x * (long)blockDim.x) {
    float4 p = p4[i], mm = m4[i], vv = v4[i];
    const uint2 gv = grad[i];
    const u16* gh = reinterpret_cast<const u16*>(&gv);
    float g[4] = {bf2f(gh[0]) * gscale, bf2f(gh[1]) * gscale,
                  bf2f(gh[2]) * gscale, bf2f(gh[3]) * gscale};
    float* pp = reinterpret_cast<float*>(&p);
    float* mp = reinterpret_cast<float*>(&mm);
    float* vp = reinterpret_cast<float*>(&vv);
    u16 outh[4];
#pragma unroll
    for (int j = 0; j < 4; ++j) {
      mp[j] = beta1 * mp[j] + (1.f - beta1) * g[j];
      vp[j] = beta2 * vp[j] + (1.f - beta2) * g[j] * g[j];
      const float mhat = mp[j] / bc1;
      const float vhat = vp[j] / bc2;
      pp[j] -= lr * (mhat / (sqrtf(vhat) + eps) + weight_decay * pp[j]);
      outh[j] = f2bf(pp[j]);
    }
    p4[i] = p; m4[i] = mm; v4[i] = vv;
    p_bf16[i] = *reinterpret_cast<uint2*>(outh);
  }
}

__global__ void adamw_bf16mom_kernel(
    float* __restrict__ p32, uint2* __restrict__ m, uint2* __restrict__ v,
    const uint2* __restrict__ grad, uint2* __restrict__ p_bf16,
    const float* __restrict__ normsq, long n4, float lr, float beta1,
    float beta2, float eps, float weight_decay, float bc1, float bc2,
    float clip, float pre_scale, const float* __restrict__ bc_dev) {
  if (bc_dev) { bc1 = bc_dev[0]; bc2 = bc_dev[1]; }
  float gscale = pre_scale;
  if (normsq) {
    const float norm = sqrtf(*normsq) * pre_scale;
    gscale = pre_scale * (clip / fmaxf(clip, norm));
  }
  float4* p4 = reinterpret_cast<float4*>(p32);
  for (long i = blockIdx.x * (long)blockDim.x + threadIdx.x; i < n4;
       i += gridDim.x * (long)blockDim.x) {
    float4 p = p4[i];
    const uint2 gv = grad[i];
    const uint2 mv = m[i];
    const uint2 vv = v[i];
    const u16* gh = reinterpret_cast<const u16*>(&gv);
    const u16* mh = reinterpret_cast<const u16*>(&mv);
    const u16* vh = reinterpret_cast<const u16*>(&vv);
    float* pp = reinterpret_cast<float*>(&p);
    u16 outp[4], outm[4], outv[4];
#pragma unroll
    for (int j = 0; j < 4; ++j) {
      const float g = bf2f(gh[j]) * gscale;
      float mj = beta1 * bf2f(mh[j]) + (1.f - beta1) * g;
      float vj = beta2 * bf2f(vh[j]) + (1.f - beta2) * g * g;
      const float mhat = mj / bc1;
      const float vhat = vj / bc2;
      pp[j] -= lr * (mhat / (sqrtf(vhat) + eps) + weight_decay * pp[j]);
      outp[j] = f2bf(pp[j]);
      outm[j] = f2bf(mj);
      outv[j] = f2bf(vj);
    }
    p4[i] = p;
    m[i] = *reinterpret_cast<uint2*>(outm);
    v[i] = *reinterpret_cast<uint2*>(outv);
    p_bf16[i] = *reinterpret_cast<uint2*>(outp);
  }
}


typedef __attribute__((ext_vector_type(8))) __bf16 bf16x8;
typedef __attribute__((ext_vector_type(4))) float f32x4;

__global__ void mfma_probe_kernel(const u16* __restrict__ A,
                                  const u16* __restrict__ B,
                                  float* __restrict__ C) {
  const int lane = threadIdx.x & 63;
  const int row = lane & 15;
  const int kg = lane >> 4;
  union { bf16x8 v; u16 h[8]; } a, b;
#pragma unroll
  for (int j = 0; j < 8; ++j) {
    a.h[j] = A[row * 32 + kg * 8 + j];
    b.h[j] = B[(kg * 8 + j) * 16 + row];
  }
  f32x4 c = {0.f, 0.f, 0.f, 0.f};
  c = __builtin_amdgcn_mfma_f32_16x16x32_bf16(a.v, b.v, c, 0, 0, 0);
#pragma unroll
  for (int r = 0; r < 4; ++r) C[(kg * 4 + r) * 16 + row] = c[r];
}


typedef __attribute__((ext_vector_type(16))) float f32x16;

__global__ void mfma_probe32_kernel(const u16* __restrict__ A,
                                    const u16* __restrict__ B,
                                    float* __restrict__ C) {
  const int lane = threadIdx.x & 63;
  const int low = lane & 31;
  const int hi = lane >> 5;
  union { bf16x8 v; u16 h[8]; } a, b;
#pragma unroll
  for (int j = 0; j < 8; ++j) {
    a.h[j] = A[low * 16 + hi * 8 + j];
    b.h[j] = B[(hi * 8 + j) * 32 + low];
  }
  f32x16 c;
#pragma unroll
  for (int r = 0; r < 16; ++r) c[r] = 0.f;
  c = __builtin_amdgcn_mfma_f32_32x32x16_bf16(a.v, b.v, c, 0, 0, 0);
#pragma unroll
  for (int r = 0; r < 16; ++r)
    C[((r & 3) + 8 * (r >> 2) + 4 * hi) * 32 + low] = c[r];
}


__global__ void tr_probe_kernel(u16* __restrict__ out, int base_elems,
                                int mode) {
  __shared__ u16 lds[4096];
  for (int i = threadIdx.x; i < 4096; i += 64) lds[i] = (u16)i;
  __syncthreads();
  const int lane = threadIdx.x & 63;
  int addr_elem = base_elems;
  if (mode == 1) addr_elem += lane;
  else if (mode == 2) addr_elem += (lane & 15);
  else if (mode == 3) addr_elem += (lane & 15) + (lane >> 4) * 64;
  const __attribute__((address_space(3))) u16* p3 =
      (const __attribute__((address_space(3))) u16*)(&lds[addr_elem]);
  unsigned long long lo;
  asm volatile("ds_read_b64_tr_b16 %0, %1\n\ts_waitcnt lgkmcnt(0)"
               : "=&v"(lo) : "v"(p3) : "memory");
  union { unsigned long long q; u16 h[4]; } u;
  u.q = lo;
#pragma unroll
  for (int j = 0; j < 4; ++j) out[lane * 4 + j] = u.h[j];
}


static inline int elementwise_grid(long nvec) {
  long g = (nvec + BLOCK - 1) / BLOCK;
  if (g > (1 << 18)) g = 1 << 18;
  if (g < 1) g = 1;
  return (int)g;
}

#define STREAM reinterpret_cast<hipStream_t>(stream)


template <int N>
__global__ __launch_bounds__(256) void gemv_bf16_kernel(
    const u16* __restrict__ w, const u16* __restrict__ x,
    u16* __restrict__ y, int M, int K) {
  const int wid = threadIdx.x >> 6;
  const int lane = threadIdx.x & 63;
  const int m = blockIdx.x * 4 + wid;
  if (m >= M) return;
  const u16* wrow = w + (long)m * K;
  float acc[N];
#pragma unroll
  for (int n = 0; n < N; ++n) acc[n] = 0.f;
  union V8 { uint4 u; u16 h[8]; };
#pragma unroll 4
  for (int c0 = lane * 8; c0 < K; c0 += 64 * 8) {
    V8 wv;
    wv.u = *reinterpret_cast<const uint4*>(wrow + c0);
#pragma unroll
    for (int n = 0; n < N; ++n) {
      V8 xv;
      xv.u = *reinterpret_cast<const uint4*>(x + (long)n * K + c0);
      float s = 0.f;
#pragma unroll
      for (int j = 0; j < 8; ++j) s += bf2f(wv.h[j]) * bf2f(xv.h[j]);
      acc[n] += s;
    }
  }
#pragma unroll
  for (int n = 0; n < N; ++n) {
#pragma unroll
    for (int off = 32; off; off >>= 1)
      acc[n] += __shfl_xor(acc[n], off, 64);
    if (lane == 0) y[(long)n * M + m] = f2bf(acc[n]);
  }
}



#define ADEC_CHUNK 64
#define ADEC_D 128

__global__ __launch_bounds__(64) void attn_decode_partial_kernel(
    const u16* __restrict__ q,
    const u16* __restrict__ kc,
    const u16* __restrict__ vc,
    const long* __restrict__ pos_dev,
    float* __restrict__ partial,
    int n_kv, int G, int Lmax, int n_chunk, float scale) {
  const int hkv = blockIdx.x / G;
  const int g = blockIdx.x % G;
  const int chunk = blockIdx.y;
  const int b = blockIdx.z;
  const int tid = threadIdx.x;
  const long pos = *pos_dev;
  __shared__ float sp[ADEC_CHUNK];
  __shared__ u16 qs[ADEC_D];
  reinterpret_cast<u32*>(qs)[tid] = reinterpret_cast<const u32*>(
      q + ((long)b * n_kv * G + hkv * G + g) * ADEC_D)[tid];
  __syncthreads();

  const long row = (long)chunk * ADEC_CHUNK + tid;
  if (row <= pos && row < Lmax) {
    const u16* krow = kc + (((long)b * n_kv + hkv) * Lmax + row) * ADEC_D;
    float sx = 0.f;
    union V8 { uint4 u; u16 h[8]; };
#pragma unroll 4
    for (int c = 0; c < ADEC_D; c += 8) {
      V8 kv8;
      kv8.u = *reinterpret_cast<const uint4*>(krow + c);
#pragma unroll
      for (int j = 0; j < 8; ++j) sx += bf2f(qs[c + j]) * bf2f(kv8.h[j]);
    }
    sp[tid] = sx * scale;
  } else {
    sp[tid] = -1e30f;
  }
  __syncthreads();

  float m = -1e30f;
  for (int r = 0; r < ADEC_CHUNK; ++r) m = fmaxf(m, sp[r]);
  const float pv = (sp[tid] > -1e30f) ? __expf(sp[tid] - m) : 0.f;
  __syncthreads();
  sp[tid] = pv;
  __syncthreads();

  const long lim = pos + 1 - (long)chunk * ADEC_CHUNK;
  const int nrow = lim < 0 ? 0 : (lim < ADEC_CHUNK ? (int)lim : ADEC_CHUNK);
  const u16* vbase = vc
      + (((long)b * n_kv + hkv) * Lmax + (long)chunk * ADEC_CHUNK) * ADEC_D
      + tid * 2;
  float a0 = 0.f, a1 = 0.f;
  for (int r = 0; r < nrow; ++r) {
    const float p = sp[r];
    union { u32 w; u16 h[2]; } vv;
    vv.w = *reinterpret_cast<const u32*>(vbase + (long)r * ADEC_D);
    a0 += p * bf2f(vv.h[0]);
    a1 += p * bf2f(vv.h[1]);
  }

  float* out = partial
      + ((((long)b * n_kv + hkv) * n_chunk + chunk) * G + g)
      * (ADEC_D + 2);
  out[tid * 2] = a0;
  out[tid * 2 + 1] = a1;
  if (tid == 0) {
    float l = 0.f;
    for (int r = 0; r < ADEC_CHUNK; ++r) l += sp[r];
    out[ADEC_D] = m;
    out[ADEC_D + 1] = l;
  }
}

__global__ __launch_bounds__(128) void attn_decode_combine_kernel(
    const float* __restrict__ partial, u16* __restrict__ o,
    int n_kv, int G, int n_chunk) {
  const int head = blockIdx.x;
  const int H = n_kv * G;
  const int b = head / H;
  const int hkv = (head % H) / G;
  const int g = head % G;
  const int tid = threadIdx.x;
  const float* base = partial
      + (((long)b * n_kv + hkv) * n_chunk * G + g) * (ADEC_D + 2);
  float M = -1e30f;
  for (int c = 0; c < n_chunk; ++c)
    M = fmaxf(M, base[(long)c * G * (ADEC_D + 2) + ADEC_D]);
  float L = 0.f, od = 0.f;
  for (int c = 0; c < n_chunk; ++c) {
    const float* pc = base + (long)c * G * (ADEC_D + 2);
    const float w = __expf(pc[ADEC_D] - M);
    L += w * pc[ADEC_D + 1];
    od += w * pc[tid];
  }
  o[(long)head * ADEC_D + tid] = f2bf(od / fmaxf(L, 1e-30f));
}


template <int N, int UNROLL, bool NT, bool W1>
__global__ __launch_bounds__(W1 ? 64 : 256) void gemv_bf16_v_kernel(
    const u16* __restrict__ w, const u16* __restrict__ x,
    u16* __restrict__ y, int M, int K) {
  const int wid = W1 ? 0 : (threadIdx.x >> 6);
  const int lane = threadIdx.x & 63;
  const int m = W1 ? blockIdx.x : blockIdx.x * 4 + wid;
  if (m >= M) return;
  const u16* wrow = w + (long)m * K;
  float acc[N];
#pragma unroll
  for (int n = 0; n < N; ++n) acc[n] = 0.f;
  typedef __attribute__((ext_vector_type(4))) unsigned int u32x4_;
  union V8 { uint4 u; u32x4_ e; u16 h[8]; };
#pragma unroll UNROLL
  for (int c0 = lane * 8; c0 < K; c0 += 64 * 8) {
    V8 wv;
    if (NT)
      wv.e = __builtin_nontemporal_load(
          reinterpret_cast<const u32x4_*>(wrow + c0));
    else
      wv.u = *reinterpret_cast<const uint4*>(wrow + c0);
#pragma unroll
    for (int n = 0; n < N; ++n) {
      V8 xv;
      xv.u = *reinterpret_cast<const uint4*>(x + (long)n * K + c0);
      float s = 0.f;
#pragma unroll
      for (int j = 0; j < 8; ++j) s += bf2f(wv.h[j]) * bf2f(xv.h[j]);
      acc[n] += s;
    }
  }
#pragma unroll
  for (int n = 0; n < N; ++n) {
#pragma unroll
    for (int off = 32; off; off >>= 1)
      acc[n] += __shfl_xor(acc[n], off, 64);
    if (lane == 0) y[(long)n * M + m] = f2bf(acc[n]);
  }
}


__global__ void rope_cache_kernel(
    const u16* __restrict__ qkv, u16* __restrict__ qout,
    u16* __restrict__ kcache, u16* __restrict__ vcache,
    const float* __restrict__ inv_freq, const long* __restrict__ pos_dev,
    int nh, int nkv, int Lmax, int D) {
  const int hx = blockIdx.x;
  const int b = blockIdx.y;
  const int d = threadIdx.x;
  const long pos = *pos_dev;
  const int half = D / 2;
  const u16* src = qkv + ((long)b * (nh + 2 * nkv)) * D + (long)hx * D;
  const float x1 = bf2f(src[d]), x2 = bf2f(src[d + half]);
  u16* dst;
  if (hx < nh) {
    dst = qout + ((long)b * nh + hx) * D;
  } else if (hx < nh + nkv) {
    dst = kcache + (((long)b * nkv + (hx - nh)) * Lmax + pos) * D;
  } else {
    vcache[(((long)b * nkv + (hx - nh - nkv)) * Lmax + pos) * D + d] =
        src[d];
    vcache[(((long)b * nkv + (hx - nh - nkv)) * Lmax + pos) * D + d
           + half] = src[d + half];
    return;
  }
  float c, sn;
  __sincosf((float)pos * inv_freq[d], &sn, &c);
  dst[d] = f2bf(x1 * c - x2 * sn);
  dst[d + half] = f2bf(x1 * sn + x2 * c);
}


template <int N>
__global__ __launch_bounds__(256) void gemv_swiglu_kernel(
    const u16* __restrict__ w, const u16* __restrict__ x,
    u16* __restrict__ y, int F, int K) {
  const int wid = threadIdx.x >> 6;
  const int lane = threadIdx.x & 63;
  const int m = blockIdx.x * 4 + wid;
  if (m >= F) return;
  const u16* grow = w + (long)m * K;
  const u16* urow = w + (long)(m + F) * K;
  float ag[N], au[N];
#pragma unroll
  for (int n = 0; n < N; ++n) ag[n] = au[n] = 0.f;
  union V8 { uint4 u; u16 h[8]; };
#pragma unroll 4
  for (int c0 = lane * 8; c0 < K; c0 += 64 * 8) {
    V8 gv, uv;
    gv.u = *reinterpret_cast<const uint4*>(grow + c0);
    uv.u = *reinterpret_cast<const uint4*>(urow + c0);
#pragma unroll
    for (int n = 0; n < N; ++n) {
      V8 xv;
      xv.u = *reinterpret_cast<const uint4*>(x + (long)n * K + c0);
#pragma unroll
      for (int j = 0; j < 8; ++j) {
        const float xf = bf2f(xv.h[j]);
        ag[n] += bf2f(gv.h[j]) * xf;
        au[n] += bf2f(uv.h[j]) * xf;
      }
    }
  }
#pragma unroll
  for (int n = 0; n < N; ++n) {
#pragma unroll
    for (int off = 32; off; off >>= 1) {
      ag[n] += __shfl_xor(ag[n], off, 64);
      au[n] += __shfl_xor(au[n], off, 64);
    }
    if (lane == 0) {
      const float g = ag[n];
      const float sg = g / (1.f + __expf(-g));
      y[(long)n * F + m] = f2bf(sg * au[n]);
    }
  }
}


__global__ __launch_bounds__(256) void gemv_moe_swiglu_kernel(
    const unsigned long long* __restrict__ table_g,
    const unsigned long long* __restrict__ table_u,
    const long* __restrict__ idx, const u16* __restrict__ x,
    u16* __restrict__ y, int F, int K, int xdiv) {
  const int wid = threadIdx.x >> 6;
  const int lane = threadIdx.x & 63;
  const int m = blockIdx.x * 4 + wid;
  const int n = blockIdx.y;
  if (m >= F) return;
  const long e = idx[n];
  const u16* grow = reinterpret_cast<const u16*>(table_g[e]) + (long)m * K;
  const u16* urow = reinterpret_cast<const u16*>(table_u[e]) + (long)m * K;
  const u16* xrow = x + (long)(n / xdiv) * K;
  float ag = 0.f, au = 0.f;
  union V8 { uint4 u; u16 h[8]; };
#pragma unroll 4
  for (int c0 = lane * 8; c0 < K; c0 += 64 * 8) {
    V8 gv, uv, xv;
    gv.u = *reinterpret_cast<const uint4*>(grow + c0);
    uv.u = *reinterpret_cast<const uint4*>(urow + c0);
    xv.u = *reinterpret_cast<const uint4*>(xrow + c0);
#pragma unroll
    for (int j = 0; j < 8; ++j) {
      const float xf = bf2f(xv.h[j]);
      ag += bf2f(gv.h[j]) * xf;
      au += bf2f(uv.h[j]) * xf;
    }
  }
#pragma unroll
  for (int off = 32; off; off >>= 1) {
    ag += __shfl_xor(ag, off, 64);
    au += __shfl_xor(au, off, 64);
  }
  if (lane == 0) {
    const float sg = ag / (1.f + __expf(-ag));
    y[(long)n * F + m] = f2bf(sg * au);
  }
}

__global__ __launch_bounds__(256) void gemv_moe_kernel(
    const unsigned long long* __restrict__ table,
    const long* __restrict__ idx, const u16* __restrict__ x,
    u16* __restrict__ y, int M, int K, int xdiv) {
  const int wid = threadIdx.x >> 6;
  const int lane = threadIdx.x & 63;
  const int m = blockIdx.x * 4 + wid;
  const int n = blockIdx.y;
  if (m >= M) return;
  const long e = idx[n];
  const u16* wrow = reinterpret_cast<const u16*>(table[e]) + (long)m * K;
  const u16* xrow = x + (long)(n / xdiv) * K;
  float acc = 0.f;
  union V8 { uint4 u; u16 h[8]; };
#pragma unroll 4
  for (int c0 = lane * 8; c0 < K; c0 += 64 * 8) {
    V8 wv, xv;
    wv.u = *reinterpret_cast<const uint4*>(wrow + c0);
    xv.u = *reinterpret_cast<const uint4*>(xrow + c0);
#pragma unroll
    for (int j = 0; j < 8; ++j) acc += bf2f(wv.h[j]) * bf2f(xv.h[j]);
  }
#pragma unroll
  for (int off = 32; off; off >>= 1) acc += __shfl_xor(acc, off, 64);
  if (lane == 0) y[(long)n * M + m] = f2bf(acc);
}

extern "C" {

int hipops_arch_check() {
  return 950;
}

void mfma_probe(void* stream, const void* A, const void* B, void* C) {
  hipLaunchKernelGGL(mfma_probe_kernel, dim3(1), dim3(64), 0, STREAM,
                     (const u16*)A, (const u16*)B, (float*)C);
}

void mfma_probe32(void* stream, const void* A, const void* B, void* C) {
  hipLaunchKernelGGL(mfma_probe32_kernel, dim3(1), dim3(64), 0, STREAM,
                     (const u16*)A, (const u16*)B, (float*)C);
}

void tr_probe(void* stream, void* out, int base_elems, int mode) {
  hipLaunchKernelGGL(tr_probe_kernel, dim3(1), dim3(64), 0, STREAM,
                     (u16*)out, base_elems, mode);
}


static inline bool rmsnorm_templated(int H) {
  const int H8 = H / 8;
  return H % 8 == 0 && H8 % BLOCK == 0 && H8 / BLOCK >= 1 && H8 / BLOCK <= 8;
}

int rmsnorm_fwd(void* stream, const void* x, const void* res_in, const void* w,
                void* y, void* res_out, void* rrms, long n_rows, int H,
                float eps) {
  if (H % 8 != 0 || H <= 0) return -1;
  if (n_rows <= 0) return 0;
  const int H8 = H / 8;
  dim3 grid((unsigned)n_rows), block(BLOCK);
  if (rmsnorm_templated(H)) {
    const int niter = H8 / BLOCK;
#define CASE(N) \
  case N: hipLaunchKernelGGL((rmsnorm_fwd_kernel<N>), grid, block, 0, STREAM, \
      (const uint4*)x, (const uint4*)res_in, (const uint4*)w, (uint4*)y, \
      (uint4*)res_out, (float*)rrms, H8, eps); return 0;
    switch (niter) {
      CASE(1) CASE(2) CASE(3) CASE(4) CASE(5) CASE(6) CASE(7) CASE(8)
    }
#undef CASE
  }
  hipLaunchKernelGGL(rmsnorm_fwd_generic_kernel, grid, block, 0, STREAM,
                     (const uint4*)x, (const uint4*)res_in, (const uint4*)w,
                     (uint4*)y, (uint4*)res_out, (float*)rrms, H8, eps);
  return 0;
}

long rmsnorm_bwd_partials(long n_rows, int H) {
  if (rmsnorm_templated(H)) return (n_rows + DW_ROWS - 1) / DW_ROWS;
  return n_rows;
}

int rmsnorm_bwd(void* stream, const void* dy, const void* res_out,
                const void* w, const void* rrms, const void* dres, void* dx,
                void* dw_partial, long n_rows, int H) {
  if (H % 8 != 0 || H <= 0) return -1;
  if (n_rows <= 0) return 0;
  const int H8 = H / 8;
  dim3 block(BLOCK);
  if (rmsnorm_templated(H)) {
    const int niter = H8 / BLOCK;
    dim3 grid((unsigned)((n_rows + DW_ROWS - 1) / DW_ROWS));
#define CASE(N) \
  case N: hipLaunchKernelGGL((rmsnorm_bwd_kernel<N>), grid, block, 0, STREAM, \
      (const uint4*)dy, (const uint4*)res_out, (const uint4*)w, \
      (const float*)rrms, (const uint4*)dres, (uint4*)dx, (float*)dw_partial, \
      n_rows, H8); return 0;
    switch (niter) {
      CASE(1) CASE(2) CASE(3) CASE(4) CASE(5) CASE(6) CASE(7) CASE(8)
    }
#undef CASE
  }
  dim3 grid((unsigned)n_rows);
  hipLaunchKernelGGL(rmsnorm_bwd_generic_kernel, grid, block, 0, STREAM,
                     (const uint4*)dy, (const uint4*)res_out, (const uint4*)w,
                     (const float*)rrms, (const uint4*)dres, (uint4*)dx,
                     (float*)dw_partial, H8);
  return 0;
}

int rmsnorm_dw_reduce(void* stream, void* dw_partial, long n_partials,
                      void* dw_f32, int H) {
  if (H <= 0 || n_partials <= 0) return -1;
  const int bx = (H + BLOCK - 1) / BLOCK;
  int ny = (1024 + bx - 1) / bx;
  if (ny < 1) ny = 1;
  if (ny > n_partials) ny = (int)n_partials;
  const int rows_per_block = (int)((n_partials + ny - 1) / ny);
  dim3 block(BLOCK);
  hipLaunchKernelGGL(rmsnorm_dw_reduce_kernel, dim3(bx, ny), block, 0, STREAM,
                     (float*)dw_partial, (int)n_partials, (float*)nullptr,
                     H, rows_per_block, 1);
  hipLaunchKernelGGL(rmsnorm_dw_reduce_kernel, dim3(bx, 1), block, 0, STREAM,
                     (float*)dw_partial, (int)n_partials, (float*)dw_f32,
                     H, (int)n_partials, rows_per_block);
  return 0;
}

int rope(void* stream, const void* x, void* out, const void* inv_freq,
         long n_tokens, int n_heads, int S, int D, float sign) {
  if (D <= 0 || D % 16 != 0 || n_heads <= 0 || S <= 0) return -1;
  if (n_tokens <= 0) return 0;
  const int vec_per_half = (D / 2) / 8;
  const long total_vec = n_tokens * (long)n_heads * vec_per_half;
  dim3 grid(elementwise_grid(total_vec)), block(BLOCK);
  hipLaunchKernelGGL(rope_kernel, grid, block, 0, STREAM, (const uint4*)x,
                     (uint4*)out, (const float*)inv_freq, total_vec,
                     vec_per_half, n_heads, S, D, sign, 0, nullptr);
  return 0;
}

int rope_at(void* stream, const void* x, void* out, const void* inv_freq,
            long n_tokens, int n_heads, int S, int D, float sign,
            int pos0) {
  if (D <= 0 || D % 16 != 0 || n_heads <= 0 || S <= 0 || pos0 < 0)
    return -1;
  if (n_tokens <= 0) return 0;
  const int vec_per_half = (D / 2) / 8;
  const long total_vec = n_tokens * (long)n_heads * vec_per_half;
  dim3 grid(elementwise_grid(total_vec)), block(BLOCK);
  hipLaunchKernelGGL(rope_kernel, grid, block, 0, STREAM, (const uint4*)x,
                     (uint4*)out, (const float*)inv_freq, total_vec,
                     vec_per_half, n_heads, S, D, sign, pos0, nullptr);
  return 0;
}

int rope_at_dev(void* stream, const void* x, void* out, const void* inv_freq,
            long n_tokens, int n_heads, int S, int D, float sign,
            const void* pos_dev) {
  if (D <= 0 || D % 16 != 0 || n_heads <= 0 || S <= 0 || !pos_dev)
    return -1;
  if (n_tokens <= 0) return 0;
  const int vec_per_half = (D / 2) / 8;
  const long total_vec = n_tokens * (long)n_heads * vec_per_half;
  dim3 grid(elementwise_grid(total_vec)), block(BLOCK);
  hipLaunchKernelGGL(rope_kernel, grid, block, 0, STREAM, (const uint4*)x,
                     (uint4*)out, (const float*)inv_freq, total_vec,
                     vec_per_half, n_heads, S, D, sign, 0, (const long*)pos_dev);
  return 0;
}


int swiglu_fwd(void* stream, const void* g, const void* u, void* out, long n) {
  if (n % 8 != 0) return -1;
  if (n == 0) return 0;
  const long n8 = n / 8;
  dim3 grid(elementwise_grid(n8)), block(BLOCK);
  hipLaunchKernelGGL(swiglu_fwd_kernel, grid, block, 0, STREAM,
                     (const uint4*)g, (const uint4*)u, (uint4*)out, n8);
  return 0;
}

int swiglu_packed_fwd(void* stream, const void* gu, void* out, long n_rows,
                      int F) {
  if (F <= 0 || F % 8 != 0) return -1;
  if (n_rows <= 0) return 0;
  const int F8 = F / 8;
  dim3 grid(elementwise_grid(n_rows * (long)F8)), block(BLOCK);
  hipLaunchKernelGGL(swiglu_packed_fwd_kernel, grid, block, 0, STREAM,
                     (const uint4*)gu, (uint4*)out, n_rows, F8);
  return 0;
}

int swiglu_packed_bwd(void* stream, const void* dout, const void* gu,
                      void* dgu, long n_rows, int F) {
  if (F <= 0 || F % 8 != 0) return -1;
  if (n_rows <= 0) return 0;
  const int F8 = F / 8;
  dim3 grid(elementwise_grid(n_rows * (long)F8)), block(BLOCK);
  hipLaunchKernelGGL(swiglu_packed_bwd_kernel, grid, block, 0, STREAM,
                     (const uint4*)dout, (const uint4*)gu, (uint4*)dgu,
                     n_rows, F8);
  return 0;
}

int swiglu_bwd(void* stream, const void* dout, const void* g, const void* u,
               void* dg, void* du, long n) {
  if (n % 8 != 0) return -1;
  if (n == 0) return 0;
  const long n8 = n / 8;
  dim3 grid(elementwise_grid(n8)), block(BLOCK);
  hipLaunchKernelGGL(swiglu_bwd_kernel, grid, block, 0, STREAM,
                     (const uint4*)dout, (const uint4*)g, (const uint4*)u,
                     (uint4*)dg, (uint4*)du, n8);
  return 0;
}

int ce_fwd(void* stream, const void* logits, const void* targets, void* lse,
           void* loss, long n_rows, int V, int ignore_index) {
  if (V <= 0 || V % 8 != 0) return -1;
  if (n_rows <= 0) return 0;
  dim3 grid((unsigned)n_rows), block(BLOCK);
  hipLaunchKernelGGL(ce_fwd_kernel, grid, block, 0, STREAM,
                     (const uint4*)logits, (const int*)targets, (float*)lse,
                     (float*)loss, V, ignore_index);
  return 0;
}

int ce_bwd(void* stream, const void* logits, const void* targets,
           const void* lse, const void* gscale, void* dlogits, long n_rows,
           int V, int ignore_index) {
  if (V <= 0 || V % 8 != 0) return -1;
  if (n_rows <= 0) return 0;
  dim3 grid((unsigned)n_rows), block(BLOCK);
  hipLaunchKernelGGL(ce_bwd_kernel, grid, block, 0, STREAM,
                     (const uint4*)logits, (const int*)targets,
                     (const float*)lse, (const float*)gscale, (uint4*)dlogits,
                     V, ignore_index);
  return 0;
}

int rows_gather(void* stream, const void* in, const void* idx, void* out,
                long n_out, int H) {
  if (H <= 0 || H % 8 != 0) return -1;
  if (n_out <= 0) return 0;
  const int H8 = H / 8;
  dim3 grid(elementwise_grid(n_out * (long)H8)), block(BLOCK);
  hipLaunchKernelGGL(rows_gather_kernel, grid, block, 0, STREAM,
                     (const uint4*)in, (const long*)idx, (uint4*)out,
                     n_out, H8);
  return 0;
}

int rows_scatter(void* stream, const void* in, const void* idx, void* out,
                 long n_in, int H) {
  if (H <= 0 || H % 8 != 0) return -1;
  if (n_in <= 0) return 0;
  const int H8 = H / 8;
  dim3 grid(elementwise_grid(n_in * (long)H8)), block(BLOCK);
  hipLaunchKernelGGL(rows_scatter_kernel, grid, block, 0, STREAM,
                     (const uint4*)in, (const long*)idx, (uint4*)out,
                     n_in, H8);
  return 0;
}

int rows_scatter_add_f32(void* stream, const void* in, const void* idx,
                         void* accum, long n_in, int H) {
  if (H <= 0 || H % 8 != 0) return -1;
  if (n_in <= 0) return 0;
  const int H8 = H / 8;
  dim3 grid(elementwise_grid(n_in * (long)H8)), block(BLOCK);
  hipLaunchKernelGGL(rows_scatter_add_f32_kernel, grid, block, 0, STREAM,
                     (const uint4*)in, (const long*)idx, (float*)accum,
                     n_in, H8);
  return 0;
}

int moe_combine(void* stream, const void* src, const void* inv,
                const void* gates, void* y, long T, int K, int H) {
  if (H <= 0 || H % 8 != 0 || K <= 0) return -1;
  if (T <= 0) return 0;
  const int H8 = H / 8;
  dim3 grid(elementwise_grid(T * (long)H8)), block(BLOCK);
  hipLaunchKernelGGL(moe_combine_kernel, grid, block, 0, STREAM,
                     (const uint4*)src, (const long*)inv,
                     (const float*)gates, (uint4*)y, T, K, H8);
  return 0;
}

int moe_combine_bwd(void* stream, const void* src, const void* dy,
                    const void* inv, const void* gates, void* dsrc,
                    void* dgate, long n_pairs, int K, int H) {
  if (H <= 0 || H % 8 != 0 || K <= 0) return -1;
  if (n_pairs <= 0) return 0;
  const int H8 = H / 8;
  dim3 grid(elementwise_grid(n_pairs * (long)H8)), block(BLOCK);
  hipLaunchKernelGGL(moe_combine_bwd_dsrc_kernel, grid, block, 0, STREAM,
                     (const uint4*)dy, (const long*)inv, (const float*)gates,
                     (uint4*)dsrc, n_pairs, K, H8);
  long gblocks = (n_pairs + (BLOCK / 16) - 1) / (BLOCK / 16);
  if (gblocks > (1 << 20)) gblocks = 1 << 20;
  hipLaunchKernelGGL(moe_combine_bwd_dgate_kernel, dim3((unsigned)gblocks),
                     block, 0, STREAM, (const uint4*)src, (const uint4*)dy,
                     (const long*)inv, (float*)dgate, n_pairs, K, H8);
  return 0;
}

int adamw_step_bf16mom(void* stream, void* p32, void* m, void* v,
                       const void* grad, void* p_bf16, const void* normsq,
                       long n, float lr, float beta1, float beta2, float eps,
                       float weight_decay, float bc1, float bc2, float clip,
                       float pre_scale, const void* bc_dev) {
  if (n % 4 != 0) return -1;
  if (n == 0) return 0;
  const long n4 = n / 4;
  dim3 grid(elementwise_grid(n4)), block(BLOCK);
  hipLaunchKernelGGL(adamw_bf16mom_kernel, grid, block, 0, STREAM,
                     (float*)p32, (uint2*)m, (uint2*)v, (const uint2*)grad,
                     (uint2*)p_bf16, (const float*)normsq, n4, lr, beta1,
                     beta2, eps, weight_decay, bc1, bc2, clip, pre_scale,
                     (const float*)bc_dev);
  return 0;
}

int l2normsq(void* stream, const void* grad, long n, void* partials,
             int n_partials, void* out) {
  if (n % 8 != 0 || n <= 0 || n_partials <= 0) return -1;
  const long n8 = n / 8;
  int grid = elementwise_grid(n8);
  if (grid > n_partials) grid = n_partials;
  hipLaunchKernelGGL(l2normsq_partial_kernel, dim3(grid), dim3(BLOCK), 0,
                     STREAM, (const uint4*)grad, n8, (float*)partials);
  hipLaunchKernelGGL(reduce_partials_kernel, dim3(1), dim3(BLOCK), 0, STREAM,
                     (const float*)partials, grid, (float*)out);
  return 0;
}

int adamw_step(void* stream, void* p32, void* m, void* v, const void* grad,
               void* p_bf16, const void* normsq, long n, float lr, float beta1,
               float beta2, float eps, float weight_decay, float bc1,
               float bc2, float clip, float pre_scale, const void* bc_dev) {
  if (n % 4 != 0) return -1;
  if (n == 0) return 0;
  const long n4 = n / 4;
  dim3 grid(elementwise_grid(n4)), block(BLOCK);
  hipLaunchKernelGGL(adamw_kernel, grid, block, 0, STREAM, (float*)p32,
                     (float*)m, (float*)v, (const uint2*)grad, (uint2*)p_bf16,
                     (const float*)normsq, n4, lr, beta1, beta2, eps,
                     weight_decay, bc1, bc2, clip, pre_scale,
                     (const float*)bc_dev);
  return 0;
}


int gemv_bf16(void* stream, const void* w, const void* x, void* y,
              int M, int K, int N) {
  if (M <= 0 || K <= 0 || (K % 512) != 0 || N < 1 || N > 8) return -1;
  if (M >= 65536) {
    dim3 grid((unsigned)M), block(64);
    switch (N) {
#define GEMV_CASE(NN) \
      case NN: \
        hipLaunchKernelGGL((gemv_bf16_v_kernel<NN, 8, true, true>), grid, \
                           block, 0, STREAM, (const u16*)w, \
                           (const u16*)x, (u16*)y, M, K); \
        break;
      GEMV_CASE(1) GEMV_CASE(2) GEMV_CASE(3) GEMV_CASE(4)
      GEMV_CASE(5) GEMV_CASE(6) GEMV_CASE(7) GEMV_CASE(8)
#undef GEMV_CASE
    }
    return 0;
  }
  dim3 grid((unsigned)((M + 3) / 4)), block(256);
  switch (N) {
#define GEMV_CASE(NN) \
    case NN: \
      hipLaunchKernelGGL((gemv_bf16_kernel<NN>), grid, block, 0, STREAM, \
                         (const u16*)w, (const u16*)x, (u16*)y, M, K); \
      break;
    GEMV_CASE(1) GEMV_CASE(2) GEMV_CASE(3) GEMV_CASE(4)
    GEMV_CASE(5) GEMV_CASE(6) GEMV_CASE(7) GEMV_CASE(8)
#undef GEMV_CASE
  }
  return 0;
}


int attn_decode(void* stream, const void* q, const void* kc,
                const void* vc, const void* pos_dev, void* partial,
                void* o, int B, int H, int n_kv, int Lmax, int n_chunk,
                float scale) {
  if (B <= 0 || n_kv <= 0 || H % n_kv != 0 ||
      n_chunk != (Lmax + ADEC_CHUNK - 1) / ADEC_CHUNK)
    return -1;
  const int G = H / n_kv;
  dim3 grid((unsigned)(n_kv * G), (unsigned)n_chunk, (unsigned)B);
  hipLaunchKernelGGL(attn_decode_partial_kernel, grid, dim3(64), 0,
                     STREAM, (const u16*)q, (const u16*)kc,
                     (const u16*)vc, (const long*)pos_dev,
                     (float*)partial, n_kv, G, Lmax, n_chunk, scale);
  hipLaunchKernelGGL(attn_decode_combine_kernel, dim3((unsigned)(B * H)),
                     dim3(128), 0, STREAM, (const float*)partial, (u16*)o,
                     n_kv, G, n_chunk);
  return 0;
}

int gemv_bf16_ab(void* stream, int which, const void* w, const void* x,
                 void* y, int M, int K) {
  if (K % 512 != 0) return -1;
  dim3 b256(256), b64(64);
  dim3 g4((unsigned)((M + 3) / 4)), g1((unsigned)M);
  switch (which) {
    case 0:
      hipLaunchKernelGGL((gemv_bf16_v_kernel<1, 4, false, false>), g4,
                         b256, 0, STREAM, (const u16*)w, (const u16*)x,
                         (u16*)y, M, K);
      break;
    case 1:
      hipLaunchKernelGGL((gemv_bf16_v_kernel<1, 8, false, false>), g4,
                         b256, 0, STREAM, (const u16*)w, (const u16*)x,
                         (u16*)y, M, K);
      break;
    case 2:
      hipLaunchKernelGGL((gemv_bf16_v_kernel<1, 8, true, false>), g4,
                         b256, 0, STREAM, (const u16*)w, (const u16*)x,
                         (u16*)y, M, K);
      break;
    case 3:
      hipLaunchKernelGGL((gemv_bf16_v_kernel<1, 8, true, true>), g1,
                         b64, 0, STREAM, (const u16*)w, (const u16*)x,
                         (u16*)y, M, K);
      break;
    default: return -1;
  }
  return 0;
}


int rope_cache(void* stream, const void* qkv, void* qout, void* kcache,
               void* vcache, const void* inv_freq, const void* pos_dev,
               int B, int nh, int nkv, int Lmax, int D) {
  if (D <= 0 || D % 16 != 0 || D / 2 > 1024 || nh <= 0 || nkv <= 0 ||
      B <= 0 || !pos_dev)
    return -1;
  dim3 grid((unsigned)(nh + 2 * nkv), (unsigned)B), block(D / 2);
  hipLaunchKernelGGL(rope_cache_kernel, grid, block, 0, STREAM,
                     (const u16*)qkv, (u16*)qout, (u16*)kcache,
                     (u16*)vcache, (const float*)inv_freq,
                     (const long*)pos_dev, nh, nkv, Lmax, D);
  return 0;
}


int gemv_swiglu(void* stream, const void* w, const void* x, void* y,
                int F, int K, int N) {
  if (F <= 0 || K <= 0 || (K % 512) != 0 || N < 1 || N > 8) return -1;
  dim3 grid((unsigned)((F + 3) / 4)), block(256);
  switch (N) {
#define GSW_CASE(NN) \
    case NN: \
      hipLaunchKernelGGL((gemv_swiglu_kernel<NN>), grid, block, 0, \
                         STREAM, (const u16*)w, (const u16*)x, (u16*)y, \
                         F, K); \
      break;
    GSW_CASE(1) GSW_CASE(2) GSW_CASE(3) GSW_CASE(4)
    GSW_CASE(5) GSW_CASE(6) GSW_CASE(7) GSW_CASE(8)
#undef GSW_CASE
  }
  return 0;
}


int gemv_moe_swiglu(void* stream, const void* table_g, const void* table_u,
                    const void* idx, const void* x, void* y,
                    int F, int K, int N, int xdiv) {
  if (F <= 0 || K <= 0 || (K % 512) != 0 || N < 1 || N > 64 || xdiv < 1)
    return -1;
  dim3 grid((unsigned)((F + 3) / 4), (unsigned)N), block(256);
  hipLaunchKernelGGL(gemv_moe_swiglu_kernel, grid, block, 0, STREAM,
                     (const unsigned long long*)table_g,
                     (const unsigned long long*)table_u,
                     (const long*)idx, (const u16*)x, (u16*)y, F, K, xdiv);
  return 0;
}

int gemv_moe(void* stream, const void* table, const void* idx,
             const void* x, void* y, int M, int K, int N, int xdiv) {
  if (M <= 0 || K <= 0 || (K % 512) != 0 || N < 1 || N > 64 || xdiv < 1)
    return -1;
  dim3 grid((unsigned)((M + 3) / 4), (unsigned)N), block(256);
  hipLaunchKernelGGL(gemv_moe_kernel, grid, block, 0, STREAM,
                     (const unsigned long long*)table,
                     (const long*)idx, (const u16*)x, (u16*)y, M, K, xdiv);
  return 0;
}

}
```

### trainingjob_operator_amd/ops/native.py

```python
from __future__ import annotations

import ctypes
import os
import subprocess
from typing import Optional

_PKG_DIR = os.path.dirname(os.path.abspath(__file__))
LIB_PATH = os.path.join(_PKG_DIR, "libhipops.so")
SRC_PATH = os.path.join(_PKG_DIR, "hip", "ops.hip")
ATTN_SRC_PATH = os.path.join(_PKG_DIR, "hip", "attention.hip")

_lib: Optional[ctypes.CDLL] = None


class HipOpsUnavailable(RuntimeError):
    pass


def build_ops(verbose: bool = False) -> str:
    cmd = [
        "hipcc", "--offload-arch=gfx950", "-O3", "-std=c++17",
        "-shared", "-fPIC", SRC_PATH, ATTN_SRC_PATH, "-o", LIB_PATH,
    ]
    if verbose:
        print("+", " ".join(cmd))
    subprocess.run(cmd, check=True)
    return LIB_PATH


def _sig(fn, argtypes, restype=None):
    fn.argtypes = argtypes
    fn.restype = restype


def load(require: bool = True) -> Optional[ctypes.CDLL]:
    global _lib
    if _lib is not None:
        return _lib
    if not os.path.exists(LIB_PATH):
        if require:
            raise HipOpsUnavailable(
                f"{LIB_PATH} not built — run trainingjob_operator_amd.ops."
                "native.build_ops() (or __graft_entry__.build())")
        return None
    lib = ctypes.CDLL(LIB_PATH)
    vp, l, i, f = ctypes.c_void_p, ctypes.c_long, ctypes.c_int, ctypes.c_float
    _sig(lib.hipops_arch_check, [], i)
    _sig(lib.rmsnorm_fwd, [vp, vp, vp, vp, vp, vp, vp, l, i, f], i)
    _sig(lib.rmsnorm_bwd, [vp, vp, vp, vp, vp, vp, vp, vp, l, i], i)
    _sig(lib.rmsnorm_bwd_partials, [l, i], l)
    _sig(lib.rmsnorm_dw_reduce, [vp, vp, l, vp, i], i)
    _sig(lib.rope, [vp, vp, vp, vp, l, i, i, i, f], i)
    _sig(lib.rope_at, [vp, vp, vp, vp, l, i, i, i, f, i], i)
    _sig(lib.rope_at_dev, [vp, vp, vp, vp, l, i, i, i, f, vp], i)
    _sig(lib.gemv_bf16, [vp, vp, vp, vp, i, i, i], i)
    _sig(lib.gemv_swiglu, [vp, vp, vp, vp, i, i, i], i)
    _sig(lib.gemv_moe_swiglu, [vp, vp, vp, vp, vp, vp, i, i, i, i], i)
    _sig(lib.gemv_moe, [vp, vp, vp, vp, vp, i, i, i, i], i)
    _sig(lib.attn_decode, [vp, vp, vp, vp, vp, vp, vp,
                           i, i, i, i, i, f], i)
    _sig(lib.rope_cache, [vp, vp, vp, vp, vp, vp, vp, i, i, i, i, i], i)
    _sig(lib.swiglu_fwd, [vp, vp, vp, vp, l], i)
    _sig(lib.swiglu_bwd, [vp, vp, vp, vp, vp, vp, l], i)
    _sig(lib.swiglu_packed_fwd, [vp, vp, vp, l, i], i)
    _sig(lib.swiglu_packed_bwd, [vp, vp, vp, vp, l, i], i)
    _sig(lib.ce_fwd, [vp, vp, vp, vp, vp, l, i, i], i)
    _sig(lib.ce_bwd, [vp, vp, vp, vp, vp, vp, l, i, i], i)
    _sig(lib.l2normsq, [vp, vp, l, vp, i, vp], i)
    _sig(lib.rows_gather, [vp, vp, vp, vp, l, i], i)
    _sig(lib.rows_scatter, [vp, vp, vp, vp, l, i], i)
    _sig(lib.rows_scatter_add_f32, [vp, vp, vp, vp, l, i], i)
    _sig(lib.moe_combine, [vp, vp, vp, vp, vp, l, i, i], i)
    _sig(lib.moe_combine_bwd, [vp, vp, vp, vp, vp, vp, vp, l, i, i], i)
    _sig(lib.adamw_step, [vp, vp, vp, vp, vp, vp, vp, l,
                          f, f, f, f, f, f, f, f, f, vp], i)
    _sig(lib.adamw_step_bf16mom, [vp, vp, vp, vp, vp, vp, vp, l,
                                  f, f, f, f, f, f, f, f, f, vp], i)
    _sig(lib.mfma_probe, [vp, vp, vp, vp])
    _sig(lib.attn_fwd, [vp, vp, vp, vp, vp, vp,
                        l, l, l, l, l, l, l, l, l, i, i, i, i, f], i)
    _sig(lib.attn_fwd_v5, [vp, vp, vp, vp, vp, vp,
                           l, l, l, l, l, l, l, l, l, i, i, i, f], i)
    _sig(lib.attn_fwd_nw8, [vp, vp, vp, vp, vp, vp,
                            l, l, l, l, l, l, l, l, l, i, i, i, i, f], i)
    _sig(lib.attn_fwd_v7, [vp, vp, vp, vp, vp, vp,
                           l, l, l, l, l, l, l, l, l, i, i, i, i, f], i)
    _sig(lib.attn_bwd, [vp, vp, vp, vp, vp, vp, vp, vp, vp, vp, vp,
                        l, l, l, l, l, l, l, l, l, i, i, i, i, f], i)
    _sig(lib.mfma_probe32, [vp, vp, vp, vp])
    assert lib.hipops_arch_check() == 950
    _lib = lib
    return lib


def check_rc(rc: int, op: str, detail: str = "") -> None:
    if rc != 0:
        raise RuntimeError(
            f"hipops {op}: unsupported shape ({detail}) — the kernel "
            f"launcher refused to launch (rc={rc})")


def available() -> bool:
    return os.path.exists(LIB_PATH)


def stream_ptr() -> ctypes.c_void_p:
    import torch
    return ctypes.c_void_p(torch.cuda.current_stream().cuda_stream)


def tr_probe_maps(device="cuda"):
    import torch
    lib = load()
    lib.tr_probe.argtypes = [ctypes.c_void_p, ctypes.c_void_p,
                             ctypes.c_int, ctypes.c_int]
    results = {}
    for mode in (0, 1, 2, 3):
        out = torch.empty(64, 4, dtype=torch.int16, device=device)
        lib.tr_probe(stream_ptr(), ctypes.c_void_p(out.data_ptr()), 0, mode)
        torch.cuda.synchronize()
        results[mode] = out.to(torch.int32).cpu() & 0xFFFF
    return results
```

Measured before the change: 17630 tokens/s.

## Fuse RoPE and attention on packed QKV with strided attention kernels

Adds a packed attention path that applies RoPE to Q and K straight out of the fused QKV projection buffer into one rotated buffer, then runs the flash attention forward and backward kernels with arbitrary strides. Attention writes its output in BSHD layout, and the backward writes dQ/dK/dV directly into a packed dQKV tensor with an inverse RoPE applied in place. This removes the split/contiguous/transpose copies and the separate per-tensor RoPE passes and their autograd overhead. It needs new strided kernel variants, and the extra stride arguments could affect register use in the hot attention kernels.

```diff
diff --git a/trainingjob_operator_amd/models/llama.py b/trainingjob_operator_amd/models/llama.py
--- a/trainingjob_operator_amd/models/llama.py
+++ b/trainingjob_operator_amd/models/llama.py
@@ -45,6 +45,17 @@
 from .config import LlamaConfig
 
 
+def _use_packed_attention(qkv: torch.Tensor, cfg: LlamaConfig) -> bool:
+    return (qkv.is_cuda and qkv.dtype == torch.bfloat16
+            and cfg.head_dim == 128 and qkv.shape[1] % 256 == 0
+            and os.environ.get("AITJ_SDPA_BACKEND", "auto") in ("auto",
+                                                                 "native")
+            and not os.environ.get("AITJ_DISABLE_GQA")
+            and os.environ.get("AITJ_ATTN_BWD") != "aten"
+            and os.environ.get("AITJ_ATTN_PACKED", "1") != "0"
+            and not fp8_enabled())
+
+
 class Attention(nn.Module):
     def __init__(self, cfg: LlamaConfig):
         super().__init__()
@@ -60,6 +71,11 @@
         B, S, H = x.shape
         cfg = self.cfg
         qkv = _proj(x, self.qkv_proj)
+        if _use_packed_attention(qkv, cfg):
+            from ..ops.attention import packed_rope_attention
+            o = packed_rope_attention(qkv, inv_freq, cfg.num_heads,
+                                      cfg.num_kv_heads)
+            return _proj(o, self.o_proj)
         q, k, v = qkv.split([self.q_size, self.kv_size, self.kv_size],
                             dim=-1)
         q = q.reshape(B, S, cfg.num_heads, cfg.head_dim).contiguous()
diff --git a/trainingjob_operator_amd/ops/attention.py b/trainingjob_operator_amd/ops/attention.py
--- a/trainingjob_operator_amd/ops/attention.py
+++ b/trainingjob_operator_amd/ops/attention.py
@@ -90,6 +90,116 @@
     return _NativeFlashAttention.apply(q, k, v, scale)
 
 
+
+def _bhsd_strides(row: int, D: int, S: int):
+    return (S * row, D, row)
+
+
+def _rope_packed(lib, x, out, inv_freq, n_tokens, n_rot, x_row, out_row,
+                 S, D, sign):
+    assert inv_freq.device == x.device and inv_freq.dtype == torch.float32, (
+        f"inv_freq must be fp32 on {x.device}, got "
+        f"{inv_freq.dtype}@{inv_freq.device}")
+    rc = lib.rope_packed(native.stream_ptr(), x.data_ptr(), out.data_ptr(),
+                         inv_freq.data_ptr(), n_tokens, n_rot, x_row,
+                         out_row, S, D, sign)
+    native.check_rc(rc, "rope_packed", f"D={D} n_rot={n_rot} row={x_row}")
+
+
+class _PackedRopeAttention(torch.autograd.Function):
+
+    @staticmethod
+    def forward(ctx, qkv, inv_freq, n_heads, n_kv_heads, scale):
+        B, S, W = qkv.shape
+        D = 128
+        H, HKV = n_heads, n_kv_heads
+        assert W == (H + 2 * HKV) * D
+        qkv = qkv.contiguous()
+        lib = native.load(require=True)
+        R = (H + HKV) * D
+        rot = torch.empty(B, S, R, dtype=torch.bfloat16, device=qkv.device)
+        _rope_packed(lib, qkv, rot, inv_freq, B * S, H + HKV, W, R, S, D, 1.0)
+        o = torch.empty(B, S, H * D, dtype=torch.bfloat16, device=qkv.device)
+        lse = torch.empty(B, H, S, dtype=torch.float32, device=qkv.device)
+        esz = qkv.element_size()
+        st = native.stride_array(
+            _bhsd_strides(R, D, S), _bhsd_strides(R, D, S),
+            _bhsd_strides(W, D, S), _bhsd_strides(H * D, D, S))
+        rc = lib.attn_fwd_strided(
+            native.stream_ptr(), rot.data_ptr(),
+            rot.data_ptr() + H * D * esz,
+            qkv.data_ptr() + (H + HKV) * D * esz,
+            o.data_ptr(), lse.data_ptr(), st, B, H, HKV, S, scale)
+        native.check_rc(rc, "attn_fwd_strided", f"B={B} H={H} HKV={HKV} S={S}")
+        ctx.save_for_backward(rot, qkv, o, lse, inv_freq)
+        ctx.dims = (B, S, H, HKV, D)
+        ctx.scale = scale
+        return o
+
+    @staticmethod
+    def backward(ctx, gout):
+        rot, qkv, o, lse, inv_freq = ctx.saved_tensors
+        B, S, H, HKV, D = ctx.dims
+        W, R = (H + 2 * HKV) * D, (H + HKV) * D
+        lib = native.load(require=True)
+        dout = gout if gout.is_contiguous() else gout.contiguous()
+        delta = torch.empty(B, H, S, dtype=torch.float32, device=qkv.device)
+        dqkv = torch.empty(B, S, W, dtype=torch.bfloat16, device=qkv.device)
+        esz = qkv.element_size()
+        rs, ws, os_ = (_bhsd_strides(R, D, S), _bhsd_strides(W, D, S),
+                       _bhsd_strides(H * D, D, S))
+        st = native.stride_array(rs, rs, ws, os_, os_, ws, ws, ws)
+        rc = lib.attn_bwd_strided(
+            native.stream_ptr(), rot.data_ptr(),
+            rot.data_ptr() + H * D * esz,
+            qkv.data_ptr() + (H + HKV) * D * esz,
+            o.data_ptr(), dout.data_ptr(), lse.data_ptr(), delta.data_ptr(),
+            dqkv.data_ptr(), dqkv.data_ptr() + H * D * esz,
+            dqkv.data_ptr() + (H + HKV) * D * esz,
+            st, B, H, HKV, S, ctx.scale)
+        native.check_rc(rc, "attn_bwd_strided", f"B={B} H={H} HKV={HKV} S={S}")
+        _rope_packed(lib, dqkv, dqkv, inv_freq, B * S, H + HKV, W, W, S, D,
+                     -1.0)
+        return dqkv, None, None, None, None
+
+
+def packed_supported(qkv: torch.Tensor, n_heads: int, n_kv_heads: int) -> bool:
+    return (qkv.is_cuda and qkv.dtype == torch.bfloat16 and qkv.dim() == 3
+            and qkv.shape[1] % 256 == 0 and n_heads % n_kv_heads == 0
+            and qkv.shape[2] == (n_heads + 2 * n_kv_heads) * 128)
+
+
+def unpacked_rope_attention(qkv, inv_freq, n_heads, n_kv_heads, scale=None):
+    from .functional import apply_rope
+    B, S, W = qkv.shape
+    D = W // (n_heads + 2 * n_kv_heads)
+    q, k, v = qkv.split([n_heads * D, n_kv_heads * D, n_kv_heads * D], dim=-1)
+    q = q.reshape(B, S, n_heads, D).contiguous()
+    k = k.reshape(B, S, n_kv_heads, D).contiguous()
+    v = v.reshape(B, S, n_kv_heads, D)
+    q = apply_rope(q, inv_freq, S).transpose(1, 2)
+    k = apply_rope(k, inv_freq, S).transpose(1, 2)
+    v = v.transpose(1, 2)
+    if qkv.is_cuda and _supported(q, k):
+        o = flash_attention(q, k, v, scale)
+    else:
+        o = torch.nn.functional.scaled_dot_product_attention(
+            q, k, v, is_causal=True, scale=scale,
+            enable_gqa=n_heads != n_kv_heads)
+    return o.transpose(1, 2).reshape(B, S, n_heads * D)
+
+
+def packed_rope_attention(qkv: torch.Tensor, inv_freq: torch.Tensor,
+                          n_heads: int, n_kv_heads: int,
+                          scale: Optional[float] = None) -> torch.Tensor:
+    if packed_supported(qkv, n_heads, n_kv_heads):
+        if scale is None:
+            scale = 1.0 / math.sqrt(128)
+        return _PackedRopeAttention.apply(qkv, inv_freq, n_heads, n_kv_heads,
+                                          scale)
+    return unpacked_rope_attention(qkv, inv_freq, n_heads, n_kv_heads, scale)
+
+
 def flash_attention_fwd_only(q, k, v, scale=None):
     if scale is None:
         scale = 1.0 / math.sqrt(q.shape[-1])
diff --git a/trainingjob_operator_amd/ops/hip/attention.hip b/trainingjob_operator_amd/ops/hip/attention.hip
--- a/trainingjob_operator_amd/ops/hip/attention.hip
+++ b/trainingjob_operator_amd/ops/hip/attention.hip
@@ -485,7 +485,33 @@
     long q_sb, long q_sh, long q_ss,
     long k_sb, long k_sh, long k_ss,
     long v_sb, long v_sh, long v_ss,
+    long o_sb, long o_sh, long o_ss,
     int n_heads, int gqa_group, int S, float scale2);
+
+static inline bool attn_strides_ok(const long* st, int n) {
+  for (int i = 0; i < n; ++i)
+    if (st[i] < 0 || st[i] % 8 != 0) return false;
+  return true;
+}
+
+static void launch_fwd_v7(void* stream, const void* q, const void* k,
+                          const void* v, void* out, void* lse,
+                          long q_sb, long q_sh, long q_ss,
+                          long k_sb, long k_sh, long k_ss,
+                          long v_sb, long v_sh, long v_ss,
+                          long o_sb, long o_sh, long o_ss,
+                          int batch, int n_heads, int n_kv_heads, int S,
+                          float scale) {
+  const float scale2 = scale * 1.4426950408889634f;
+  dim3 grid(S / 256, n_heads, batch), block(512);
+  hipLaunchKernelGGL(attn_fwd_v7_kernel, grid, block, 0,
+                     reinterpret_cast<hipStream_t>(stream),
+                     (const u16*)q, (const u16*)k, (const u16*)v,
+                     (u16*)out, (float*)lse, q_sb, q_sh, q_ss,
+                     k_sb, k_sh, k_ss, v_sb, v_sh, v_ss,
+                     o_sb, o_sh, o_ss, n_heads,
+                     n_heads / n_kv_heads, S, scale2);
+}
 
 extern "C" int attn_fwd(void* stream, const void* q, const void* k,
                         const void* v, void* out, void* lse,
@@ -500,13 +526,10 @@
   if (S % 128 == 0) {
     const float scale2 = scale * 1.4426950408889634f;
     if (S % 256 == 0) {
-      dim3 grid(S / 256, n_heads, batch), block(512);
-      hipLaunchKernelGGL(attn_fwd_v7_kernel, grid, block, 0,
-                         reinterpret_cast<hipStream_t>(stream),
-                         (const u16*)q, (const u16*)k, (const u16*)v,
-                         (u16*)out, (float*)lse, q_sb, q_sh, q_ss,
-                         k_sb, k_sh, k_ss, v_sb, v_sh, v_ss, n_heads,
-                         n_heads / n_kv_heads, S, scale2);
+      launch_fwd_v7(stream, q, k, v, out, lse, q_sb, q_sh, q_ss,
+                    k_sb, k_sh, k_ss, v_sb, v_sh, v_ss,
+                    (long)n_heads * S * ATTN_D, (long)S * ATTN_D, ATTN_D,
+                    batch, n_heads, n_kv_heads, S, scale);
       return 0;
     }
     dim3 grid(S / 128, n_heads, batch), block(256);
@@ -566,13 +589,21 @@
 
 __global__ __launch_bounds__(256) void attn_delta_kernel(
     const u16* __restrict__ dout, const u16* __restrict__ o,
-    float* __restrict__ delta, long n_rows) {
-  const long row = (long)blockIdx.x * 16 + (threadIdx.x >> 4);
-  if (row >= n_rows) return;
+    float* __restrict__ delta,
+    long do_sb, long do_sh, long do_ss,
+    long o_sb, long o_sh, long o_ss,
+    int n_heads, int S) {
+  const int s = blockIdx.x * 16 + (threadIdx.x >> 4);
+  const int h = blockIdx.y;
+  const int bi = blockIdx.z;
+  if (s >= S) return;
+  const long row = ((long)bi * n_heads + h) * S + s;
   const int e8 = (threadIdx.x & 15) * 8;
   union { uint4 u; u16 h[8]; } a, b;
-  a.u = *reinterpret_cast<const uint4*>(dout + row * ATTN_D + e8);
-  b.u = *reinterpret_cast<const uint4*>(o + row * ATTN_D + e8);
+  a.u = *reinterpret_cast<const uint4*>(
+      dout + (long)bi * do_sb + (long)h * do_sh + (long)s * do_ss + e8);
+  b.u = *reinterpret_cast<const uint4*>(
+      o + (long)bi * o_sb + (long)h * o_sh + (long)s * o_ss + e8);
   float acc = 0.f;
 #pragma unroll
   for (int j = 0; j < 8; ++j)
@@ -596,6 +627,8 @@
     long q_sb, long q_sh, long q_ss,
     long k_sb, long k_sh, long k_ss,
     long v_sb, long v_sh, long v_ss,
+    long do_sb, long do_sh, long do_ss,
+    long dq_sb, long dq_sh, long dq_ss,
     int n_heads, int gqa_group, int S, float scale) {
   constexpr int NT = 512;
   const int qb = gridDim.x - 1 - blockIdx.x;
@@ -621,7 +654,8 @@
 
   union F8 { bf16x8 v; uint4 u; u16 h[8]; };
   const u16* qptr = q + (long)b * q_sb + (long)h * q_sh + (long)qrow * q_ss;
-  const u16* doptr = dout + (((long)b * n_heads + h) * S + qrow) * ATTN_D;
+  const u16* doptr = dout + (long)b * do_sb + (long)h * do_sh
+                     + (long)qrow * do_ss;
   F8 qf[8], dof[8];
 #pragma unroll
   for (int kc = 0; kc < 8; ++kc) {
@@ -766,7 +800,7 @@
     v7_barrier();
   }
 
-  u16* dqrow = dq + (((long)b * n_heads + h) * S + qrow) * ATTN_D;
+  u16* dqrow = dq + (long)b * dq_sb + (long)h * dq_sh + (long)qrow * dq_ss;
 #pragma unroll
   for (int ds = 0; ds < 4; ++ds) {
 #pragma unroll
@@ -796,6 +830,8 @@
     u16* __restrict__ dv,
     long q_sb, long q_sh, long q_ss,
     long k_sb, long k_sh, long k_ss,
+    long do_sb, long do_sh, long do_ss,
+    long dv_sb, long dv_sh, long dv_ss,
     int n_heads, int n_kv_heads, int S, float scale) {
   const int kvb = blockIdx.x;
   const int hkv = blockIdx.y;
@@ -838,7 +874,7 @@
   for (int g = 0; g < gqa_group; ++g) {
     const int h = hkv * gqa_group + g;
     const u16* qbase = q + (long)b * q_sb + (long)h * q_sh;
-    const u16* dobase = dout + (((long)b * n_heads + h) * S) * ATTN_D;
+    const u16* dobase = dout + (long)b * do_sb + (long)h * do_sh;
     const float* lbase = lse + ((long)b * n_heads + h) * S;
 
     const u16* qgp[2];
@@ -853,11 +889,11 @@
       qgp[1] = qbase + (long)(qt0 * 64 + r1) * q_ss + in1;
       const int rp2 = (tid >> 4) * 2;
       const int c8 = (tid & 15) * 8;
-      dtp[0] = dobase + (long)(qt0 * 64 + rp2) * ATTN_D + c8;
-      dtp[1] = dobase + (long)(qt0 * 64 + rp2 + 1) * ATTN_D + c8;
+      dtp[0] = dobase + (long)(qt0 * 64 + rp2) * do_ss + c8;
+      dtp[1] = dobase + (long)(qt0 * 64 + rp2 + 1) * do_ss + c8;
     }
     const long qstep = (long)64 * q_ss;
-    const long dostep = (long)64 * ATTN_D;
+    const long dostep = (long)64 * do_ss;
 
 #define BV_STAGE_IN(BUFI, QT)                                               \
     {                                                                       \
@@ -967,7 +1003,7 @@
     }
   }
 
-  u16* dvrow = dv + (((long)b * n_kv_heads + hkv) * S + kvrow) * ATTN_D;
+  u16* dvrow = dv + (long)b * dv_sb + (long)hkv * dv_sh + (long)kvrow * dv_ss;
 #pragma unroll
   for (int ds = 0; ds < 4; ++ds) {
 #pragma unroll
@@ -1001,6 +1037,8 @@
     long q_sb, long q_sh, long q_ss,
     long k_sb, long k_sh, long k_ss,
     long v_sb, long v_sh, long v_ss,
+    long do_sb, long do_sh, long do_ss,
+    long dk_sb, long dk_sh, long dk_ss,
     int n_heads, int n_kv_heads, int S, float scale) {
   const int kvb = blockIdx.x;
   const int hkv = blockIdx.y;
@@ -1048,7 +1086,7 @@
   for (int g = 0; g < gqa_group; ++g) {
     const int h = hkv * gqa_group + g;
     const u16* qbase = q + (long)b * q_sb + (long)h * q_sh;
-    const u16* dobase = dout + (((long)b * n_heads + h) * S) * ATTN_D;
+    const u16* dobase = dout + (long)b * do_sb + (long)h * do_sh;
     const float* lbase = lse + ((long)b * n_heads + h) * S;
     const float* dbase = delta + ((long)b * n_heads + h) * S;
 
@@ -1063,15 +1101,15 @@
       const int in1 = (((L1 & 255) ^ ((r1 & 15) << 4)) >> 1);
       qgp[0] = qbase + (long)(qt0 * 64 + r0) * q_ss + in0;
       qgp[1] = qbase + (long)(qt0 * 64 + r1) * q_ss + in1;
-      dgp[0] = dobase + (long)(qt0 * 64 + r0) * ATTN_D + in0;
-      dgp[1] = dobase + (long)(qt0 * 64 + r1) * ATTN_D + in1;
+      dgp[0] = dobase + (long)(qt0 * 64 + r0) * do_ss + in0;
+      dgp[1] = dobase + (long)(qt0 * 64 + r1) * do_ss + in1;
       const int rp2 = (tid >> 4) * 2;
       const int c8 = (tid & 15) * 8;
       qtp[0] = qbase + (long)(qt0 * 64 + rp2) * q_ss + c8;
       qtp[1] = qbase + (long)(qt0 * 64 + rp2 + 1) * q_ss + c8;
     }
     const long qstep = (long)64 * q_ss;
-    const long dostep = (long)64 * ATTN_D;
+    const long dostep = (long)64 * do_ss;
 
 #define BK_STAGE_IN(BUFI, QT)                                               \
     {                                                                       \
@@ -1196,7 +1234,7 @@
     }
   }
 
-  u16* dkrow = dk + (((long)b * n_kv_heads + hkv) * S + kvrow) * ATTN_D;
+  u16* dkrow = dk + (long)b * dk_sb + (long)hkv * dk_sh + (long)kvrow * dk_ss;
 #pragma unroll
   for (int ds = 0; ds < 4; ++ds) {
 #pragma unroll
@@ -1217,6 +1255,61 @@
 
 
 
+struct AttnStride { long sb, sh, ss; };
+
+static inline AttnStride attn_dense_stride(int n_heads, int S) {
+  return {(long)n_heads * S * ATTN_D, (long)S * ATTN_D, (long)ATTN_D};
+}
+
+static int launch_bwd(void* stream, const void* q, const void* k,
+                      const void* v, const void* out, const void* dout,
+                      const void* lse, void* delta,
+                      void* dq, void* dk, void* dv,
+                      AttnStride qs, AttnStride ks, AttnStride vs,
+                      AttnStride os, AttnStride dos,
+                      AttnStride dqs, AttnStride dks, AttnStride dvs,
+                      int batch, int n_heads, int n_kv_heads, int S,
+                      float scale) {
+  if (S <= 0 || S % 256 != 0 || n_heads <= 0 || batch <= 0 ||
+      n_kv_heads <= 0 || n_heads % n_kv_heads != 0)
+    return -1;
+  hipStream_t st = reinterpret_cast<hipStream_t>(stream);
+  hipLaunchKernelGGL(attn_delta_kernel, dim3(S / 16, n_heads, batch),
+                     dim3(256), 0, st,
+                     (const u16*)dout, (const u16*)out, (float*)delta,
+                     dos.sb, dos.sh, dos.ss, os.sb, os.sh, os.ss,
+                     n_heads, S);
+  {
+    dim3 grid(S / 256, n_heads, batch), block(512);
+    hipLaunchKernelGGL(attn_bwd_dq_kernel, grid, block, 0, st,
+                       (const u16*)q, (const u16*)k, (const u16*)v,
+                       (const u16*)dout, (const float*)lse,
+                       (const float*)delta, (u16*)dq,
+                       qs.sb, qs.sh, qs.ss, ks.sb, ks.sh, ks.ss,
+                       vs.sb, vs.sh, vs.ss, dos.sb, dos.sh, dos.ss,
+                       dqs.sb, dqs.sh, dqs.ss,
+                       n_heads, n_heads / n_kv_heads, S, scale);
+  }
+  {
+    dim3 grid(S / 256, n_kv_heads, batch), block(512);
+    hipLaunchKernelGGL(attn_bwd_dv_kernel, grid, block, 0, st,
+                       (const u16*)q, (const u16*)k, (const u16*)dout,
+                       (const float*)lse, (u16*)dv,
+                       qs.sb, qs.sh, qs.ss, ks.sb, ks.sh, ks.ss,
+                       dos.sb, dos.sh, dos.ss, dvs.sb, dvs.sh, dvs.ss,
+                       n_heads, n_kv_heads, S, scale);
+    hipLaunchKernelGGL(attn_bwd_dk_kernel, grid, block, 0, st,
+                       (const u16*)q, (const u16*)k, (const u16*)v,
+                       (const u16*)dout, (const float*)lse,
+                       (const float*)delta, (u16*)dk,
+                       qs.sb, qs.sh, qs.ss, ks.sb, ks.sh, ks.ss,
+                       vs.sb, vs.sh, vs.ss, dos.sb, dos.sh, dos.ss,
+                       dks.sb, dks.sh, dks.ss,
+                       n_heads, n_kv_heads, S, scale);
+  }
+  return 0;
+}
+
 extern "C" int attn_bwd(void* stream, const void* q, const void* k,
                         const void* v, const void* out, const void* dout,
                         const void* lse, void* delta,
@@ -1226,40 +1319,27 @@
                         long v_sb, long v_sh, long v_ss,
                         int batch, int n_heads, int n_kv_heads, int S,
                         float scale) {
-  if (S <= 0 || S % 256 != 0 || n_heads <= 0 || batch <= 0 ||
-      n_kv_heads <= 0 || n_heads % n_kv_heads != 0)
-    return -1;
-  hipStream_t st = reinterpret_cast<hipStream_t>(stream);
-  const long n_rows = (long)batch * n_heads * S;
-  hipLaunchKernelGGL(attn_delta_kernel,
-                     dim3((unsigned)((n_rows + 15) / 16)), dim3(256), 0, st,
-                     (const u16*)dout, (const u16*)out, (float*)delta,
-                     n_rows);
-  {
-    dim3 grid(S / 256, n_heads, batch), block(512);
-    hipLaunchKernelGGL(attn_bwd_dq_kernel, grid, block, 0, st,
-                       (const u16*)q, (const u16*)k, (const u16*)v,
-                       (const u16*)dout, (const float*)lse,
-                       (const float*)delta, (u16*)dq,
-                       q_sb, q_sh, q_ss, k_sb, k_sh, k_ss,
-                       v_sb, v_sh, v_ss, n_heads, n_heads / n_kv_heads, S,
-                       scale);
-  }
-  {
-    dim3 grid(S / 256, n_kv_heads, batch), block(512);
-    hipLaunchKernelGGL(attn_bwd_dv_kernel, grid, block, 0, st,
-                       (const u16*)q, (const u16*)k, (const u16*)dout,
-                       (const float*)lse, (u16*)dv,
-                       q_sb, q_sh, q_ss, k_sb, k_sh, k_ss,
-                       n_heads, n_kv_heads, S, scale);
-    hipLaunchKernelGGL(attn_bwd_dk_kernel, grid, block, 0, st,
-                       (const u16*)q, (const u16*)k, (const u16*)v,
-                       (const u16*)dout, (const float*)lse,
-                       (const float*)delta, (u16*)dk,
-                       q_sb, q_sh, q_ss, k_sb, k_sh, k_ss,
-                       v_sb, v_sh, v_ss, n_heads, n_kv_heads, S, scale);
-  }
-  return 0;
+  const AttnStride dh = attn_dense_stride(n_heads, S);
+  const AttnStride dkv = attn_dense_stride(n_kv_heads, S);
+  return launch_bwd(stream, q, k, v, out, dout, lse, delta, dq, dk, dv,
+                    {q_sb, q_sh, q_ss}, {k_sb, k_sh, k_ss},
+                    {v_sb, v_sh, v_ss}, dh, dh, dh, dkv, dkv,
+                    batch, n_heads, n_kv_heads, S, scale);
+}
+
+extern "C" int attn_bwd_strided(void* stream, const void* q, const void* k,
+                                const void* v, const void* out,
+                                const void* dout, const void* lse,
+                                void* delta, void* dq, void* dk, void* dv,
+                                const long* st, int batch, int n_heads,
+                                int n_kv_heads, int S, float scale) {
+  if (!st || !attn_strides_ok(st, 24)) return -1;
+  auto tri = [st](int i) {
+    return AttnStride{st[3 * i], st[3 * i + 1], st[3 * i + 2]};
+  };
+  return launch_bwd(stream, q, k, v, out, dout, lse, delta, dq, dk, dv,
+                    tri(0), tri(1), tri(2), tri(3), tri(4), tri(5), tri(6),
+                    tri(7), batch, n_heads, n_kv_heads, S, scale);
 }
 
 
@@ -1270,6 +1350,7 @@
     long q_sb, long q_sh, long q_ss,
     long k_sb, long k_sh, long k_ss,
     long v_sb, long v_sh, long v_ss,
+    long o_sb, long o_sh, long o_ss,
     int n_heads, int gqa_group, int S, float scale2) {
   constexpr int NT = 512;
   const int qb = gridDim.x - 1 - blockIdx.x;
@@ -1476,7 +1557,7 @@
   }
 
   const float inv_l = 1.0f / l_run;
-  u16* orow = out + (((long)b * n_heads + h) * S + qrow) * ATTN_D;
+  u16* orow = out + (long)b * o_sb + (long)h * o_sh + (long)qrow * o_ss;
 #pragma unroll
   for (int ds = 0; ds < 4; ++ds) {
 #pragma unroll
@@ -1505,13 +1586,23 @@
                            int batch, int n_heads, int n_kv_heads, int S,
                            float scale) {
   if (S <= 0 || S % 256 != 0 || n_heads % n_kv_heads != 0) return -1;
-  dim3 grid(S / 256, n_heads, batch), block(512);
-  const float scale2 = scale * 1.4426950408889634f;
-  hipLaunchKernelGGL(attn_fwd_v7_kernel, grid, block, 0,
-                     reinterpret_cast<hipStream_t>(stream),
-                     (const u16*)q, (const u16*)k, (const u16*)v, (u16*)out,
-                     (float*)lse, q_sb, q_sh, q_ss, k_sb, k_sh, k_ss,
-                     v_sb, v_sh, v_ss, n_heads, n_heads / n_kv_heads, S,
-                     scale2);
+  launch_fwd_v7(stream, q, k, v, out, lse, q_sb, q_sh, q_ss,
+                k_sb, k_sh, k_ss, v_sb, v_sh, v_ss,
+                (long)n_heads * S * ATTN_D, (long)S * ATTN_D, ATTN_D,
+                batch, n_heads, n_kv_heads, S, scale);
   return 0;
 }
+
+extern "C" int attn_fwd_strided(void* stream, const void* q, const void* k,
+                                const void* v, void* out, void* lse,
+                                const long* st, int batch, int n_heads,
+                                int n_kv_heads, int S, float scale) {
+  if (S <= 0 || S % 256 != 0 || n_heads <= 0 || batch <= 0 ||
+      n_kv_heads <= 0 || n_heads % n_kv_heads != 0)
+    return -1;
+  if (!st || !attn_strides_ok(st, 12)) return -1;
+  launch_fwd_v7(stream, q, k, v, out, lse, st[0], st[1], st[2],
+                st[3], st[4], st[5], st[6], st[7], st[8],
+                st[9], st[10], st[11], batch, n_heads, n_kv_heads, S, scale);
+  return 0;
+}
diff --git a/trainingjob_operator_amd/ops/hip/ops.hip b/trainingjob_operator_amd/ops/hip/ops.hip
--- a/trainingjob_operator_amd/ops/hip/ops.hip
+++ b/trainingjob_operator_amd/ops/hip/ops.hip
@@ -284,6 +284,23 @@
   else if (p0 < n_partials) dw_partial[(long)p0 * H + h] = acc;
 }
 
+
+__device__ __forceinline__ void rope_rotate8(const BF8& a, const BF8& b,
+                                             BF8& oa, BF8& ob,
+                                             const float* inv_freq, int i0,
+                                             int pos, float sign) {
+#pragma clang fp contract(off)
+#pragma unroll
+  for (int j = 0; j < 8; ++j) {
+    float c, s;
+    __sincosf((float)pos * inv_freq[i0 + j], &s, &c);
+    s *= sign;
+    const float x1 = bf2f(a.h[j]), x2 = bf2f(b.h[j]);
+    const float x2s = x2 * s, x2c = x2 * c;
+    oa.h[j] = f2bf(__builtin_fmaf(x1, c, -x2s));
+    ob.h[j] = f2bf(__builtin_fmaf(x1, s, x2c));
+  }
+}
 
 __global__ void rope_kernel(const uint4* __restrict__ x, uint4* __restrict__ out,
                             const float* __restrict__ inv_freq,
@@ -303,17 +320,35 @@
     BF8 a; a.v = x[base + i0 / 8];
     BF8 b; b.v = x[base + (HALF + i0) / 8];
     BF8 oa, ob;
-#pragma unroll
-    for (int j = 0; j < 8; ++j) {
-      float c, s;
-      __sincosf((float)pos * inv_freq[i0 + j], &s, &c);
-      s *= sign;
-      const float x1 = bf2f(a.h[j]), x2 = bf2f(b.h[j]);
-      oa.h[j] = f2bf(x1 * c - x2 * s);
-      ob.h[j] = f2bf(x1 * s + x2 * c);
-    }
+    rope_rotate8(a, b, oa, ob, inv_freq, i0, pos, sign);
     out[base + i0 / 8] = oa.v;
     out[base + (HALF + i0) / 8] = ob.v;
+  }
+}
+
+__global__ void rope_packed_kernel(const uint4* x, uint4* out,
+                                   const float* __restrict__ inv_freq,
+                                   long total_vec, int vec_per_half,
+                                   int n_rot, long x_row_vec,
+                                   long out_row_vec, int S, int D,
+                                   float sign) {
+  const int HALF = D / 2;
+  for (long g = blockIdx.x * (long)blockDim.x + threadIdx.x; g < total_vec;
+       g += gridDim.x * (long)blockDim.x) {
+    const long per_head = vec_per_half;
+    const long head_g = g / per_head;
+    const int i0 = (int)(g % per_head) * 8;
+    const long t = head_g / n_rot;
+    const int h = (int)(head_g % n_rot);
+    const int pos = (int)(t % S);
+    const long xb = t * x_row_vec + (long)h * (D / 8);
+    const long ob_ = t * out_row_vec + (long)h * (D / 8);
+    BF8 a; a.v = x[xb + i0 / 8];
+    BF8 b; b.v = x[xb + (HALF + i0) / 8];
+    BF8 oa, ob;
+    rope_rotate8(a, b, oa, ob, inv_freq, i0, pos, sign);
+    out[ob_ + i0 / 8] = oa.v;
+    out[ob_ + (HALF + i0) / 8] = ob.v;
   }
 }
 
@@ -1255,6 +1290,24 @@
   hipLaunchKernelGGL(rope_kernel, grid, block, 0, STREAM, (const uint4*)x,
                      (uint4*)out, (const float*)inv_freq, total_vec,
                      vec_per_half, n_heads, S, D, sign, 0, (const long*)pos_dev);
+  return 0;
+}
+
+int rope_packed(void* stream, const void* x, void* out, const void* inv_freq,
+                long n_tokens, int n_rot, long x_row, long out_row, int S,
+                int D, float sign) {
+  if (D <= 0 || D % 16 != 0 || n_rot <= 0 || S <= 0) return -1;
+  if (x_row % 8 != 0 || out_row % 8 != 0 || x_row < (long)n_rot * D ||
+      out_row < (long)n_rot * D)
+    return -1;
+  if (n_tokens <= 0) return 0;
+  const int vec_per_half = (D / 2) / 8;
+  const long total_vec = n_tokens * (long)n_rot * vec_per_half;
+  dim3 grid(elementwise_grid(total_vec)), block(BLOCK);
+  hipLaunchKernelGGL(rope_packed_kernel, grid, block, 0, STREAM,
+                     (const uint4*)x, (uint4*)out, (const float*)inv_freq,
+                     total_vec, vec_per_half, n_rot, x_row / 8, out_row / 8,
+                     S, D, sign);
   return 0;
 }
 
diff --git a/trainingjob_operator_amd/ops/native.py b/trainingjob_operator_amd/ops/native.py
--- a/trainingjob_operator_amd/ops/native.py
+++ b/trainingjob_operator_amd/ops/native.py
@@ -53,6 +53,7 @@
     _sig(lib.rope, [vp, vp, vp, vp, l, i, i, i, f], i)
     _sig(lib.rope_at, [vp, vp, vp, vp, l, i, i, i, f, i], i)
     _sig(lib.rope_at_dev, [vp, vp, vp, vp, l, i, i, i, f, vp], i)
+    _sig(lib.rope_packed, [vp, vp, vp, vp, l, i, l, l, i, i, f], i)
     _sig(lib.gemv_bf16, [vp, vp, vp, vp, i, i, i], i)
     _sig(lib.gemv_swiglu, [vp, vp, vp, vp, i, i, i], i)
     _sig(lib.gemv_moe_swiglu, [vp, vp, vp, vp, vp, vp, i, i, i, i], i)
@@ -87,6 +88,10 @@
                            l, l, l, l, l, l, l, l, l, i, i, i, i, f], i)
     _sig(lib.attn_bwd, [vp, vp, vp, vp, vp, vp, vp, vp, vp, vp, vp,
                         l, l, l, l, l, l, l, l, l, i, i, i, i, f], i)
+    lp = ctypes.POINTER(ctypes.c_long)
+    _sig(lib.attn_fwd_strided, [vp, vp, vp, vp, vp, vp, lp, i, i, i, i, f], i)
+    _sig(lib.attn_bwd_strided, [vp, vp, vp, vp, vp, vp, vp, vp, vp, vp, vp,
+                                lp, i, i, i, i, f], i)
     _sig(lib.mfma_probe32, [vp, vp, vp, vp])
     assert lib.hipops_arch_check() == 950
     _lib = lib
@@ -98,6 +103,12 @@
         raise RuntimeError(
             f"hipops {op}: unsupported shape ({detail}) — the kernel "
             f"launcher refused to launch (rc={rc})")
+
+
+def stride_array(*triples):
+    flat = [int(x) for t in triples for x in t]
+    assert len(flat) == 3 * len(triples)
+    return (ctypes.c_long * len(flat))(*flat)
 
 
 def available() -> bool:
```

After: 17990 tokens/s, median of 6. 1.02x the previous value.
